# YoungSean/UnseenObjectsWithMeanShift

Measured on AMD Instinct MI355X. Metric: images/sec @640x480 RGB-D, 100 queries, 9 decoder layers; % MFMA roofline, higher is better.
Workload: dtype f32; 1 GPU; configs[1]: batch 8 of 640x480 per GPU, ResNet-50 features -> MSDeformAttn pixel decoder -> 9-layer decoder, 100 q ->~; global_batch=8, per_gpu_batch=8, launch=hipgraph x4: 4 batches of 8 in flight, one graph + stream each, batches_in_flight=4, parallelism=dp1, GPU_MAX_HW_QUEUES=4, visible_gpus=1, rank0_numa=pinned

## Files before the change

include/msm_hip.h:

```cpp
#ifndef MSM_HIP_H
#define MSM_HIP_H

#include <stdint.h>

#ifdef __cplusplus
extern "C" {
#endif

#define MSM_OK 0
#define MSM_E_INVALID (-1)
#define MSM_E_LAUNCH (-2)
#define MSM_E_WORKSPACE (-3)

const char* msm_last_error_string(void);
#define MSM_ABI_VERSION 28
int msm_abi_version(void);

#define MSM_OPT_AUTO (-1)
enum {
    MSM_OPT_MASK_NC = 0,
    MSM_OPT_MASKB_TARGET,
    MSM_OPT_GEMM_TILE,
    MSM_OPT_GEMM_SHALLOW,
    MSM_OPT_ATTN_TARGET,
    MSM_OPT_ATTN_KERNEL,
    MSM_OPT_ATTN_QK_MAX,
    MSM_OPT_ATTN_QKCFG,
    MSM_OPT_CONVIN_NT,
    MSM_OPT_POST_GENERIC,
    MSM_OPT_ENC_NO_COOP,
    MSM_OPT_MSDA_GENERIC,
    MSM_OPT_MS_CHUNK,
    MSM_OPT_MS_NO_PERSISTENT,
    MSM_OPT_ATTN_FUSED_KV,
    MSM_OPT_KV_PIPE,
    MSM_OPT_MASK_KERNEL,
    MSM_OPT_MS_SPLIT_KERNEL,
    MSM_OPT_CONV3_WIDE,
    MSM_OPT_DEC_TILE32,
    MSM_OPT_POST_RESIZE_DIRECT,
    MSM_OPT_COUNT
};
int msm_set_option(int key, int value);
int msm_get_option(int key);

int msm_gemm_f32(const float* A, const float* A2, const float* W, const float* bias, float* C,
                 int M, int N, int K, int batch,
                 int64_t a_sm, int64_t a_sk, int64_t a_sb, int64_t a2_sb, int64_t w_sb,
                 int64_t c_sm, int64_t c_sn, int64_t c_sb, int64_t c_ss,
                 int a_mode, int conv_h, int conv_w, int conv_c,
                 int bias_mode, int act, int split_k, void* stream);

int msm_layernorm_f32(const float* x, const float* parts, int n_parts, int64_t part_stride,
                      const float* bias, const float* g1, const float* b1, int l2norm,
                      const float* g2, const float* b2, float* y, float* y2,
                      int rows, int E, float eps, void* stream);

int msm_groupnorm_stats_f32(const float* x, double* stats, int stats_cleared, int B, int HW, int C, void* stream);
int msm_groupnorm_apply_f32(const float* x, const double* stats, const float* gamma, const float* beta,
                            const float* up, int uh, int uw, int64_t up_batch_stride, float* y,
                            int B, int H, int W, int C, int groups, float eps, int relu, void* stream);

int msm_groupnorm_apply_split(const float* x, const double* stats, const float* gamma, const float* beta,
                              const float* up, int uh, int uw, int64_t up_batch_stride, uint16_t* planes,
                              int B, int H, int W, int C, int groups, float eps, int relu, void* stream);

int msm_groupnorm_apply_f16(const float* x, const double* stats, const float* gamma, const float* beta,
                            const float* up, int uh, int uw, int64_t up_batch_stride, void* y_f16,
                            int B, int H, int W, int C, int groups, float eps, int relu, void* stream);

int msm_groupnorm_apply_nchw_f32(const float* x, const double* stats, const float* gamma, const float* beta, float* y,
                                 int B, int HW, int C, int groups, float eps, int relu, void* stream);

int msm_pos_embed_sine(float* out, int H, int W, int npf, int64_t s_c, int64_t s_p,
                       const float* add_c, float temperature, float scale, void* stream);

int msm_transpose_f32(const float* in, float* out, int B, int R, int C, void* stream);

int msm_l2_normalize_nchw_f32(const float* x, float* y, int B, int C, int HW, float eps, void* stream);

int msm_msda_locations(const float* offsets, const float* logits, const float* reference_points, const int64_t* spatial_shapes,
                       float* sampling_loc, float* attn_weight, int64_t rows, int M, int L, int P, void* stream);

#define MSM_MASK_SPARSE 1
#define MSM_MASK_ROW_ANY_CLEARED 2
#define MSM_MASK_F16 4
int msm_mask_logits_fwd(const float* mask_embed, const float* mask_feat, float* mask_out,
                        uint8_t* attn_out, int32_t* row_any,
                        int B, int Q, int C, int H, int W, int th, int tw, int flags,
                        int64_t embed_ld, const float* qbias, int64_t qbias_ld, void* stream);

int msm_pack_mask_features_bf16(const float* mask_feat, uint16_t* packed, int B, int C, int HW, void* stream);
int msm_pack_mask_features_f16(const float* mask_feat, uint16_t* packed, int B, int C, int HW, void* stream);
int msm_mask_logits_bf16_fwd(const float* mask_embed, const uint16_t* mask_feat_packed, float* mask_out,
                             uint8_t* attn_out, int32_t* row_any,
                             int B, int Q, int C, int H, int W, int th, int tw, int flags,
                             int64_t embed_ld, const float* qbias, int64_t qbias_ld, void* stream);

int msm_pack_mask_features_split(const float* mask_feat, uint16_t* packed, int B, int C, int HW, void* stream);
int msm_mask_logits_split_fwd(const float* mask_embed, const uint16_t* mask_feat_split, float* mask_out,
                              uint8_t* attn_out, int32_t* row_any, int B, int Q, int C, int H, int W, int th, int tw,
                              int flags, int64_t embed_ld, const float* qbias, int64_t qbias_ld, void* stream);

int64_t msm_hypersphere_attn_workspace(int B, int Lq, int S, int heads);
int msm_hypersphere_attn_fwd(const float* q, const float* k, const float* v,
                             const uint8_t* masked, const int32_t* row_any, float* out,
                             int B, int Lq, int S, int heads,
                             int64_t ldq, int64_t q_sb, int64_t ldk, int64_t k_sb,
                             int64_t ldv, int64_t v_sb, float kappa,
                             float* workspace, int64_t workspace_elems, void* stream);
int msm_hypersphere_attn_lp_fwd(const float* q, const void* k, const void* v, int kv_format,
                                const uint8_t* masked, const int32_t* row_any, float* out,
                                int B, int Lq, int S, int heads,
                                int64_t ldq, int64_t q_sb, int64_t ldk, int64_t k_sb,
                                int64_t ldv, int64_t v_sb, float kappa,
                                float* workspace, int64_t workspace_elems, void* stream);

int msm_nchw_to_tokens_f16(const float* in, void* out, int B, int C, int HW, void* stream);
int msm_attn_pack_kv_weights(const float* w, void* packed, int heads, void* stream);
int msm_mask_conv3x3_folded(const void* x_f16, const float* F, int64_t ldf, int64_t f_sb, void* mask_bits, int32_t* row_any, int row_any_cleared,
                            float* logits, int B, int Q, int H, int W, void* stream);
int64_t msm_attn_mask_bits_bytes(int B, int Lq, int S);
int msm_attn_pack_mask_bits(const uint8_t* masked, void* bits, int B, int Lq, int S, void* stream);
int msm_hypersphere_attn_fused_kv_fwd(const float* q, const void* x_f16, const void* w_packed, const float* rowcol, const float* col_v_t,
                                      int score_format, const void* mask_bits, const int32_t* row_any, float* out,
                                      int B, int Lq, int H, int W, int heads, int64_t ldq, int64_t q_sb, float kappa,
                                      float* workspace, int64_t workspace_elems, void* stream);

int msm_msdeform_attn_fwd(const float* value, const int64_t* spatial_shapes,
                          const int64_t* level_start_index, const float* sampling_loc,
                          const float* attn_weight, float* out,
                          int B, int S, int M, int D, int L, int Lq, int P, void* stream);

int msm_msdeform_attn_bwd(const float* value, const int64_t* spatial_shapes,
                          const int64_t* level_start_index, const float* sampling_loc,
                          const float* attn_weight, const float* grad_output,
                          float* grad_value, float* grad_sampling_loc, float* grad_attn_weight,
                          int B, int S, int M, int D, int L, int Lq, int P, void* stream);
int msm_msdeform_attn_fwd_f64(const double* value, const int64_t* spatial_shapes,
                              const int64_t* level_start_index, const double* sampling_loc,
                              const double* attn_weight, double* out,
                              int B, int S, int M, int D, int L, int Lq, int P, void* stream);
int msm_msdeform_attn_bwd_f64(const double* value, const int64_t* spatial_shapes,
                              const int64_t* level_start_index, const double* sampling_loc,
                              const double* attn_weight, const double* grad_output,
                              double* grad_value, double* grad_sampling_loc, double* grad_attn_weight,
                              int B, int S, int M, int D, int L, int Lq, int P, void* stream);

int msm_msdeform_attn_enc_fwd(const float* value, const int64_t* spatial_shapes,
                              const int64_t* level_start_index, const float* proj, float* out,
                              int B, int S, int M, int D, int L, int P, void* stream);

int msm_value_to_head_major_f32(const float* value, float* value_hm, int B, int S, int M, int D, void* stream);
int msm_msdeform_attn_enc_hm_fwd(const float* value_hm, const int64_t* spatial_shapes,
                                 const int64_t* level_start_index, const float* proj, float* out,
// ... 293 lines not shown
```

unseenobjectswithmeanshift_amd/_lib.py:

```python
import ctypes
import os
import re

_HERE = os.path.dirname(os.path.abspath(__file__))
LIB_PATH = os.path.join(_HERE, "libmsm_hip.so")
HEADER_PATH = os.path.join(os.path.dirname(_HERE), "include", "msm_hip.h")

_lib = None
ABI_VERSION = 28

c_f = ctypes.c_void_p
c_p = ctypes.c_void_p
c_i = ctypes.c_int
c_l = ctypes.c_int64
c_fl = ctypes.c_float

_SIGNATURES = {
    "msm_abi_version": (c_i, []),
    "msm_last_error_string": (ctypes.c_char_p, []),
    "msm_set_option": (c_i, [c_i, c_i]),
    "msm_get_option": (c_i, [c_i]),
    "msm_gemm_f32": (c_i, [c_f, c_f, c_f, c_f, c_f, c_i, c_i, c_i, c_i,
                           c_l, c_l, c_l, c_l, c_l, c_l, c_l, c_l, c_l,
                           c_i, c_i, c_i, c_i, c_i, c_i, c_i, c_p]),
    "msm_layernorm_f32": (c_i, [c_f, c_f, c_i, c_l, c_f, c_f, c_f, c_i, c_f, c_f, c_f, c_f, c_i, c_i, c_fl, c_p]),
    "msm_groupnorm_stats_f32": (c_i, [c_f, c_p, c_i, c_i, c_i, c_i, c_p]),
    "msm_groupnorm_apply_f32": (c_i, [c_f, c_p, c_f, c_f, c_f, c_i, c_i, c_l, c_f, c_i, c_i, c_i, c_i, c_i, c_fl, c_i, c_p]),
    "msm_groupnorm_apply_split": (c_i, [c_f, c_p, c_f, c_f, c_f, c_i, c_i, c_l, c_f, c_i, c_i, c_i, c_i, c_i, c_fl, c_i, c_p]),
    "msm_groupnorm_apply_f16": (c_i, [c_f, c_p, c_f, c_f, c_f, c_i, c_i, c_l, c_p, c_i, c_i, c_i, c_i, c_i, c_fl, c_i, c_p]),
    "msm_groupnorm_apply_nchw_f32": (c_i, [c_f, c_p, c_f, c_f, c_f, c_i, c_i, c_i, c_i, c_fl, c_i, c_p]),
    "msm_pos_embed_sine": (c_i, [c_f, c_i, c_i, c_i, c_l, c_l, c_f, c_fl, c_fl, c_p]),
    "msm_transpose_f32": (c_i, [c_f, c_f, c_i, c_i, c_i, c_p]),
    "msm_l2_normalize_nchw_f32": (c_i, [c_f, c_f, c_i, c_i, c_i, c_fl, c_p]),
    "msm_msda_locations": (c_i, [c_f, c_f, c_f, c_p, c_f, c_f, c_l, c_i, c_i, c_i, c_p]),
    "msm_mask_logits_fwd": (c_i, [c_f, c_f, c_f, c_p, c_p, c_i, c_i, c_i, c_i, c_i, c_i, c_i, c_i, c_l, c_f, c_l, c_p]),
    "msm_pool_mask_taps": (c_i, [c_f, c_i, c_i, c_i, c_i, c_p, c_p, c_p, c_p, c_l, c_p]),
    "msm_attn_mask_pooled": (c_i, [c_f, c_l, c_f, c_l, c_f, c_p, c_p, c_i, c_i, c_i, c_i, c_i, c_p]),
    "msm_pack_mask_features_bf16": (c_i, [c_f, c_p, c_i, c_i, c_i, c_p]),
    "msm_pack_mask_features_f16": (c_i, [c_f, c_p, c_i, c_i, c_i, c_p]),
    "msm_mask_logits_bf16_fwd": (c_i, [c_f, c_p, c_f, c_p, c_p, c_i, c_i, c_i, c_i, c_i, c_i, c_i, c_i, c_l, c_f, c_l, c_p]),
    "msm_pack_mask_features_split": (c_i, [c_f, c_p, c_i, c_i, c_i, c_p]),
    "msm_mask_logits_split_fwd": (c_i, [c_f, c_p, c_f, c_p, c_p, c_i, c_i, c_i, c_i, c_i, c_i, c_i, c_i, c_l, c_f, c_l, c_p]),
    "msm_hypersphere_attn_workspace": (c_l, [c_i, c_i, c_i, c_i]),
    "msm_hypersphere_attn_fwd": (c_i, [c_f, c_f, c_f, c_p, c_p, c_f, c_i, c_i, c_i, c_i,
                                       c_l, c_l, c_l, c_l, c_l, c_l, c_fl, c_f, c_l, c_p]),
    "msm_hypersphere_attn_lp_fwd": (c_i, [c_f, c_p, c_p, c_i, c_p, c_p, c_f, c_i, c_i, c_i, c_i,
                                          c_l, c_l, c_l, c_l, c_l, c_l, c_fl, c_f, c_l, c_p]),
    "msm_hypersphere_attn_bwd_workspace": (c_l, [c_i, c_i, c_i]),
    "msm_hypersphere_attn_bwd": (c_i, [c_f, c_f, c_f, c_p, c_p, c_f, c_f, c_f, c_f, c_i, c_i, c_i, c_i,
                                       c_l, c_l, c_l, c_l, c_l, c_l, c_fl, c_f, c_l, c_p]),
    "msm_msdeform_attn_fwd": (c_i, [c_f, c_p, c_p, c_f, c_f, c_f, c_i, c_i, c_i, c_i, c_i, c_i, c_i, c_p]),
    "msm_msdeform_attn_bwd": (c_i, [c_f, c_p, c_p, c_f, c_f, c_f, c_f, c_f, c_f, c_i, c_i, c_i, c_i, c_i, c_i, c_i, c_p]),
    "msm_msdeform_attn_fwd_f64": (c_i, [c_f, c_p, c_p, c_f, c_f, c_f, c_i, c_i, c_i, c_i, c_i, c_i, c_i, c_p]),
    "msm_msdeform_attn_bwd_f64": (c_i, [c_f, c_p, c_p, c_f, c_f, c_f, c_f, c_f, c_f, c_i, c_i, c_i, c_i, c_i, c_i, c_i, c_p]),
    "msm_msdeform_attn_enc_fwd": (c_i, [c_f, c_p, c_p, c_f, c_f, c_i, c_i, c_i, c_i, c_i, c_i, c_p]),
    "msm_encoder_block_stream_floats": (c_l, [c_i, c_i]),
    "msm_value_to_head_major_f32": (c_i, [c_f, c_f, c_i, c_i, c_i, c_i, c_p]),
    "msm_msdeform_attn_enc_hm_fwd": (c_i, [c_f, c_p, c_p, c_f, c_f, c_i, c_i, c_i, c_i, c_i, c_i, c_p]),
    "msm_msda_pack_proj": (c_i, [c_f, c_f, c_f, c_f, c_i, c_i, c_i, c_p]),
    "msm_msdeform_attn_enc_fused_fwd": (c_i, [c_f, c_p, c_p, c_f, c_f, c_f, c_f, c_f, c_i, c_i, c_i, c_i, c_i, c_i, c_p]),
    "msm_encoder_block_fwd": (c_i, [c_f, c_f, c_f, c_f, c_f, c_f, c_f, c_f, c_i, c_i, c_i, c_i, c_i, c_fl, c_p]),
    "msm_encoder_block_split_stream_bytes": (c_l, [c_i, c_i]),
    "msm_encoder_block_split_fwd": (c_i, [c_f, c_f, c_p, c_f, c_f, c_f, c_f, c_f, c_i, c_i, c_i, c_i, c_i, c_fl, c_p]),
    "msm_encoder_block_lp_stream_bytes": (c_l, [c_i, c_i]),
    "msm_encoder_block_lp_fwd": (c_i, [c_f, c_f, c_p, c_f, c_f, c_f, c_f, c_f, c_i, c_i, c_i, c_i, c_i, c_fl, c_p]),
    "msm_encoder_block_hm_stream_bytes": (c_l, [c_i, c_i]),
    "msm_encoder_block_hm_small_floats": (c_i, [c_i]),
    "msm_encoder_block_hm_fwd": (c_i, [c_p, c_f, c_p, c_f, c_f, c_f, c_p, c_p, c_i, c_i, c_i, c_fl, c_i, c_p]),
    "msm_msdeform_attn_enc_lp_fwd": (c_i, [c_p, c_p, c_p, c_p, c_p, c_i, c_i, c_i, c_i, c_i, c_i, c_p]),
    "msm_msdeform_attn_enc_lp_fused_fwd": (c_i, [c_p, c_p, c_p, c_f, c_f, c_p, c_f, c_p, c_i, c_i, c_i, c_i, c_i, c_i, c_p]),
    "msm_f32_to_f16": (c_i, [c_f, c_p, c_l, c_p]),
    "msm_bias_act_nhwc": (c_i, [c_p, c_p, c_p, c_i, c_l, c_i, c_i, c_p]),
    "msm_nhwc_to_nchw_f32": (c_i, [c_p, c_f, c_i, c_i, c_i, c_i, c_p]),
    "msm_ucn_embedding_tail": (c_i, [c_f, c_f, c_f, c_i, c_i, c_i, c_i, c_i, c_i, c_fl, c_p]),
    "msm_f32_to_f16_rows": (c_i, [c_f, c_p, c_i, c_l, c_l, c_p]),
    "msm_kv_project_f32": (c_i, [c_f, c_f, c_f, c_f, c_i, c_i, c_i, c_i, c_i, c_l, c_i, c_p]),
    "msm_kv_project_multi_f32": (c_i, [c_i, c_p, c_p, c_p, c_p, c_p, c_p, c_p, c_p, c_i, c_i, c_i, c_p]),
    "msm_kv_project_multi_bf16": (c_i, [c_i, c_p, c_p, c_p, c_p, c_p, c_p, c_p, c_p, c_i, c_i, c_i, c_i, c_p]),
    "msm_kv_project_multi_split": (c_i, [c_i, c_p, c_p, c_p, c_p, c_p, c_p, c_p, c_p, c_i, c_i, c_i, c_p]),
    "msm_tokens_proj_nchw_f32": (c_i, [c_f, c_f, c_f, c_p, c_f, c_f, c_i, c_fl, c_i, c_f, c_i, c_i, c_i, c_i, c_p]),
    "msm_dec_pack_weight": (c_i, [c_f, c_f, c_i, c_i, c_p]),
    "msm_dec_post_cross": (c_i, [c_f] * 12 + [c_i, c_i, c_i, c_fl, c_p]),
    "msm_dec_post_self": (c_i, [c_f] * 9 + [c_i, c_f, c_f, c_i, c_i, c_i, c_fl, c_p]),
    "msm_dec_heads": (c_i, [c_f, c_f, c_i, c_f, c_f, c_f, c_i] + [c_f] * 15 + [c_p, c_i, c_i, c_i, c_fl, c_p]),
    "msm_dec_pack_weight_bf16": (c_i, [c_f, c_p, c_i, c_i, c_p]),
    "msm_dec_post_cross_bf16": (c_i, [c_f, c_f, c_f, c_p, c_f, c_f, c_f, c_p, c_f, c_f, c_f, c_f] + [c_i, c_i, c_i, c_fl, c_p]),
    "msm_dec_post_self_bf16": (c_i, [c_f, c_f, c_p, c_f, c_f, c_f, c_p, c_f, c_p] + [c_i, c_f, c_f, c_i, c_i, c_i, c_fl, c_p]),
    "msm_dec_heads_bf16": (c_i, [c_f, c_f, c_i, c_f, c_f, c_f, c_i, c_f, c_f, c_p, c_f, c_p, c_f, c_p, c_f, c_p, c_f, c_f] + [c_f] * 4 +
                           [c_p, c_i, c_i, c_i, c_fl, c_p]),
    "msm_nchw_to_tokens_f16": (c_i, [c_f, c_p, c_i, c_i, c_i, c_p]),
    "msm_mask_conv3x3_folded": (c_i, [c_p, c_f, c_l, c_l, c_p, c_p, c_i, c_f, c_i, c_i, c_i, c_i, c_p]),
    "msm_attn_pack_kv_weights": (c_i, [c_f, c_p, c_i, c_p]),
    "msm_attn_mask_bits_bytes": (c_l, [c_i, c_i, c_i]),
    "msm_attn_pack_mask_bits": (c_i, [c_p, c_p, c_i, c_i, c_i, c_p]),
    "msm_hypersphere_attn_fused_kv_fwd": (c_i, [c_f, c_p, c_p, c_f, c_f, c_i, c_p, c_p, c_f, c_i, c_i, c_i, c_i, c_i, c_l, c_l, c_fl, c_f, c_l, c_p]),
    "msm_dec_pack_weight_f16": (c_i, [c_f, c_p, c_i, c_i, c_p]),
    "msm_dec_post_cross_f16": (c_i, [c_f, c_f, c_f, c_p, c_f, c_f, c_f, c_p, c_f, c_f, c_f, c_f] + [c_i, c_i, c_i, c_fl, c_p]),
    "msm_dec_post_self_f16": (c_i, [c_f, c_f, c_p, c_f, c_f, c_f, c_p, c_f, c_p] + [c_i, c_f, c_f, c_i, c_i, c_i, c_fl, c_p]),
    "msm_dec_heads_f16": (c_i, [c_f, c_f, c_i, c_f, c_f, c_f, c_i, c_f, c_f, c_p, c_f, c_p, c_f, c_p, c_f, c_p, c_f, c_f] + [c_f] * 4 +
                          [c_p, c_i, c_i, c_i, c_fl, c_p]),
    "msm_dec_heads_mask": (c_i, [c_f, c_f, c_i, c_f, c_f, c_f, c_i, c_f, c_f, c_p, c_f, c_p, c_f, c_p, c_f, c_p, c_f, c_f] + [c_f] * 4 +
                           [c_f, c_i, c_i, c_p, c_p, c_i, c_i, c_i, c_i, c_fl, c_p]),
    "msm_dec_pack_weight_bf16x2": (c_i, [c_f, c_p, c_i, c_i, c_p]),
    "msm_dec_post_cross_bf16x2": (c_i, [c_f, c_f, c_f, c_p, c_f, c_f, c_f, c_p, c_f, c_f, c_f, c_f] + [c_i, c_i, c_i, c_fl, c_p]),
    "msm_dec_post_self_bf16x2": (c_i, [c_f, c_f, c_p, c_f, c_f, c_f, c_p, c_f, c_p] + [c_i, c_f, c_f, c_i, c_i, c_i, c_fl, c_p]),
    "msm_dec_heads_bf16x2": (c_i, [c_f, c_f, c_i, c_f, c_f, c_f, c_i, c_f, c_f, c_p, c_f, c_p, c_f, c_p, c_f, c_p, c_f, c_f] + [c_f] * 4 +
                             [c_p, c_i, c_i, c_i, c_fl, c_p]),
    "msm_l2_prefetch": (c_i, [c_p, c_p, c_i, c_p]),
    "msm_dec_set_prefetch": (c_i, [c_p, c_p, c_i]),
    "msm_ms_seed_workspace": (c_l, [c_i]),
    "msm_ms_select_seeds": (c_i, [c_f, c_i, c_i, c_i, c_l, c_f, c_p, c_f, c_l, c_i, c_p]),
    "msm_ms_hill_climb_workspace": (c_l, [c_i, c_i]),
    "msm_ms_hill_climb": (c_i, [c_f, c_i, c_i, c_f, c_i, c_fl, c_i, c_f, c_l, c_p]),
# ... 1 lines not shown
    "msm_ms_hill_climb_split": (c_i, [c_f, c_i, c_i, c_f, c_i, c_fl, c_i, c_f, c_l, c_p]),
    "msm_ms_bf16_rows": (c_l, [c_i]),
    "msm_ms_pack_bf16": (c_i, [c_f, c_i, c_i, c_p, c_p]),
    "msm_ms_select_seeds_bf16": (c_i, [c_p, c_f, c_i, c_i, c_i, c_l, c_f, c_p, c_f, c_l, c_i, c_p]),
    "msm_ms_hill_climb_bf16": (c_i, [c_p, c_i, c_i, c_f, c_i, c_fl, c_i, c_f, c_l, c_p]),
    "msm_ms_assign": (c_i, [c_f, c_i, c_i, c_f, c_i, c_p, c_p, c_p, c_i, c_p]),
    "msm_ms_connected_components": (c_i, [c_f, c_i, c_i, c_fl, c_p, c_p, c_p]),
    "msm_ms_relabel_largest_zero": (c_i, [c_p, c_i, c_p, c_i, c_p, c_p]),
    "msm_ms_seed_batched_workspace": (c_l, [c_i, c_i]),
    "msm_ms_select_seeds_batched": (c_i, [c_f, c_i, c_i, c_i, c_i, c_p, c_f, c_p, c_f, c_l, c_i, ctypes.c_uint64, c_p]),
    "msm_ms_hill_climb_batched_workspace": (c_l, [c_i, c_i, c_i]),
    "msm_ms_hill_climb_batched": (c_i, [c_f, c_i, c_i, c_i, c_f, c_i, c_fl, c_i, c_f, c_l, c_p]),
    "msm_ms_assign_batched": (c_i, [c_f, c_i, c_i, c_i, c_f, c_i, c_p, c_p, c_p, c_i, c_p]),
    "msm_ms_connected_components_batched": (c_i, [c_f, c_i, c_i, c_i, c_fl, c_p, c_p, c_p]),
    "msm_ms_relabel_largest_zero_batched": (c_i, [c_p, c_i, c_i, c_p, c_i, c_p, c_p]),
    "msm_topk_class_scores": (c_i, [c_f, c_i, c_i, c_i, c_i, c_f, c_p, c_p, c_p]),
    "msm_topk_class_scores_gather": (c_i, [c_f, c_i, c_i, c_i, c_i, c_f, c_p, c_p, c_f, c_l, c_i, c_f, c_p]),
    "msm_conv1x1_in_f32": (c_i, [c_f, c_f, c_f, c_f, c_l, c_p, c_i, c_i, c_i, c_i, c_p]),
    "msm_conv1x1_in_multi_f32": (c_i, [c_i, c_p, c_p, c_p, c_p, c_p, c_f, c_l, c_p, c_i, c_i, c_p]),
    "msm_conv1x1_in_multi_lp": (c_i, [c_i, c_p, c_p, c_p, c_p, c_p, c_f, c_l, c_p, c_i, c_i, c_p]),
    "msm_conv1x1_in_multi_wide": (c_i, [c_i, c_p, c_p, c_p, c_p, c_p, c_f, c_l, c_p, c_i, c_i, c_p]),
    "msm_conv1x1_in_lp": (c_i, [c_f, c_p, c_f, c_f, c_l, c_p, c_i, c_i, c_i, c_i, c_p]),
    "msm_conv3x3_c64_f32": (c_i, [c_f, c_f, c_f, c_p, c_i, c_i, c_i, c_i, c_p]),
    "msm_conv3x3_c64_bf16": (c_i, [c_f, c_f, c_f, c_p, c_i, c_i, c_i, c_i, c_p]),
    "msm_conv3x3_c64_f16": (c_i, [c_f, c_f, c_f, c_p, c_i, c_i, c_i, c_i, c_p]),
    "msm_conv3x3_c64_f16h": (c_i, [c_p, c_f, c_f, c_p, c_i, c_i, c_i, c_i, c_p]),
    "msm_conv3x3_c64_nchw_f16": (c_i, [c_f, c_f, c_f, c_f, c_i, c_i, c_i, c_i, c_p]),
    "msm_conv3x3_c64_split": (c_i, [c_f, c_f, c_f, c_p, c_i, c_i, c_i, c_i, c_p]),
    "msm_conv3x3_c64_nchw_f32": (c_i, [c_f, c_f, c_f, c_f, c_i, c_i, c_i, c_i, c_p]),
    "msm_conv3x3_c64_nchw_bf16": (c_i, [c_f, c_f, c_f, c_f, c_i, c_i, c_i, c_i, c_p]),
    "msm_encoder_prologue_stream_floats": (c_l, [c_i]),
    "msm_encoder_prologue_fwd": (c_i, [c_f, c_p, c_f, c_p, c_i, c_i, c_fl, c_f, c_f, c_f, c_f, c_p, c_p, c_i, c_i, c_i, c_i, c_i, c_p]),
    "msm_encoder_prologue_hm_weight_bytes": (c_l, []),
    "msm_encoder_prologue_hm_fwd": (c_i, [c_f, c_p, c_f, c_p, c_i, c_i, c_fl, c_p, c_f, c_f, c_f, c_p, c_p, c_i, c_i, c_p]),
    "msm_label_stats": (c_i, [c_f, c_f, c_p, c_f, c_p, c_i, c_i, c_i, c_i, c_p]),
    "msm_label_image": (c_i, [c_f, c_f, c_f, c_i, c_i, c_i, c_i, c_p]),
    "msm_crop_resize": (c_i, [c_f, c_f, c_f, c_p, c_f, c_f, c_f, c_i, c_i, c_i, c_i, c_p]),
    "msm_paste_labels": (c_i, [c_f, c_p, c_p, c_p, c_f, c_i, c_i, c_i, c_i, c_p]),
    "msm_mask_nms_workspace": (c_l, [c_i, c_i, c_i, c_i]),
    "msm_mask_nms": (c_i, [c_f, c_f, c_p, c_fl, c_f, c_f, c_f, c_p, c_p, c_p, c_l, c_i, c_i, c_i, c_i, c_p]),
    "msm_ingest_frames": (c_i, [c_p, c_p, c_i, c_fl, c_f, c_f, c_f, c_f, c_i, c_i, c_i, c_i, c_i, c_i, c_p]),
    "msm_instance_postprocess_workspace": (c_l, [c_i, c_i, c_i, c_i]),
    "msm_eval_counts_workspace": (c_l, [c_i]),
    "msm_eval_counts": (c_i, [c_f, c_f, c_p, c_p, c_l, c_i, c_i, c_i, c_i, c_i, c_p]),
    "msm_match_cost": (c_i, [c_p, c_p, c_p, c_f, c_f, c_i, c_i, c_i, c_i, c_i, c_i, c_i, c_i, c_i, c_i, c_i,
                             c_fl, c_fl, c_fl, c_p]),
    "msm_point_loss_workspace": (c_l, [c_i, c_i]),
    "msm_point_loss_fwd": (c_i, [c_p, c_p, c_p, c_f, c_f, c_f, c_p, c_p, c_l, c_i, c_i, c_i, c_i, c_i, c_i, c_i, c_i,
                                 c_i, c_i, c_i, c_fl, c_p]),
    "msm_point_loss_bwd": (c_i, [c_p, c_p, c_p, c_f, c_f, c_p, c_l, c_f, c_i, c_i, c_i, c_i, c_i, c_i, c_i, c_i,
                                 c_i, c_i, c_i, c_fl, c_i, c_p]),
    "msm_instance_postprocess": (c_i, [c_f, c_p, c_f, c_f, c_f, c_f, c_i, c_i, c_i, c_i, c_i, c_i, c_i, c_i, c_i, c_f, c_p]),
    "msm_instance_postprocess_resized": (c_i, [c_f, c_p, c_f, c_f, c_f, c_f] + [c_i] * 11 + [c_f, c_p]),
}


def declared_symbols():
    with open(HEADER_PATH) as f:
        src = f.read()
    src = re.sub(r"/\*.*?\*/", "", src, flags=re.S)
    return sorted(set(re.findall(r"\b(msm_[a-z0-9_]+)\s*\(", src)))


def lib():
    global _lib
    if _lib is None:
        if not os.path.exists(LIB_PATH):
            raise RuntimeError(
                f"{LIB_PATH} is missing: build it with `python -c 'import __graft_entry__ as g; g.build()'` "
                "(hipcc --offload-arch=gfx950). There is no CPU fallback for the HIP hot path.")
        L = ctypes.CDLL(LIB_PATH)
        for name, (res, args) in _SIGNATURES.items():
            fn = getattr(L, name)
            fn.restype = res
            fn.argtypes = args
        if L.msm_abi_version() != ABI_VERSION:
            raise RuntimeError(f"{LIB_PATH} has ABI {L.msm_abi_version()}, these bindings need {ABI_VERSION}: rebuild it")
        _lib = L
    return _lib


OPTIONS = ("MASK_NC", "MASKB_TARGET", "GEMM_TILE", "GEMM_SHALLOW", "ATTN_TARGET", "ATTN_KERNEL", "ATTN_QK_MAX", "ATTN_QKCFG",
           "CONVIN_NT", "POST_GENERIC", "ENC_NO_COOP", "MSDA_GENERIC", "MS_CHUNK", "MS_NO_PERSISTENT", "ATTN_FUSED_KV", "KV_PIPE", "MASK_KERNEL",
           "MS_SPLIT_KERNEL", "CONV3_WIDE", "DEC_TILE32", "POST_RESIZE_DIRECT")
OPT_AUTO = -1


def set_option(name, value=OPT_AUTO):
    key = OPTIONS.index(name)
    old = lib().msm_get_option(key)
    check(lib().msm_set_option(key, int(value)), "msm_set_option")
    if old != int(value):
        from ._plan import bump_plan_epoch
        bump_plan_epoch()
    return old


class option:

    def __init__(self, name, value):
        self.name, self.value = name, value

    def __enter__(self):
        self.old = set_option(self.name, self.value)
        return self

    def __exit__(self, *exc):
        set_option(self.name, self.old)
        return False


class CallTimer:

    def __init__(self):
        self.records = []
        self._saved = {}

    def __enter__(self):
        import torch
        L = lib()
        for name, (_, args) in _SIGNATURES.items():
            if not args or args[-1] is not c_p or name.endswith("_workspace"):
                continue
            fn = getattr(L, name)
            self._saved[name] = fn

            def wrapped(*a, _fn=fn, _name=name):
                e0, e1 = torch.cuda.Event(enable_timing=True), torch.cuda.Event(enable_timing=True)
                e0.record()
                rc = _fn(*a)
                e1.record()
                self.records.append((_name, e0, e1))
                return rc

            setattr(L, name, wrapped)
        return self

    def __exit__(self, *exc):
        L = lib()
        for name, fn in self._saved.items():
            setattr(L, name, fn)
        self._saved = {}
        return False

    def durations(self):
        out = {}
        for name, e0, e1 in self.records:
            out.setdefault(name, []).append(e0.elapsed_time(e1))
        return out


def check(rc, what):
    if rc != 0:
        msg = lib().msm_last_error_string()
        raise RuntimeError(f"{what} failed (code {rc}): {msg.decode() if msg else ''}")
```

unseenobjectswithmeanshift_amd/csrc/mask_logits.hip:

```cpp
#include <stdlib.h>

#include <type_traits>

#include "bf16.h"
#include "common.h"

namespace msm {

constexpr int QB = 7;
constexpr int QCH = QB * 16;
#ifndef MSM_MASK_KU
#define MSM_MASK_KU 4
#endif
#ifndef MSM_WRITE_AUX
#define MSM_WRITE_AUX 0
#endif
#ifndef MSM_MASK_MW
#define MSM_MASK_MW 8
#endif
constexpr int KU = MSM_MASK_KU;
constexpr int MW = MSM_MASK_MW;

typedef unsigned int u32x2 __attribute__((ext_vector_type(2)));

#ifdef MSM_MASK_TS
__device__ unsigned long long g_mask_ts[256 * 8 * 16];
#define MASK_TS(slot)                                                                                          \
    if (lane == 0 && blockIdx.y == 0 && (int)(blockIdx.z * gridDim.x + blockIdx.x) < 256 && (slot) < 16)       \
        g_mask_ts[((blockIdx.z * gridDim.x + blockIdx.x) * 8 + wave) * 16 + (slot)] = wall_clock64();
#define MASK_TSC(slot)                                                                                         \
    if (lane == 0 && blockIdx.y == 0 && (int)(blockIdx.z * gridDim.x + blockIdx.x) < 256 && (slot) < 16)       \
        g_mask_ts[((blockIdx.z * gridDim.x + blockIdx.x) * 8 + wave) * 16 + (slot)] = clock64();
#else
#define MASK_TS(slot)
#define MASK_TSC(slot)
#endif

template <int NC>
struct Cols {
    float v[NC];
};
template <int NC>
__device__ __forceinline__ Cols<NC> ld_cols(__amdgpu_buffer_rsrc_t rsrc, unsigned voff, unsigned soff) {
    Cols<NC> c;
    if constexpr (NC == 2) {
        const u32x2 t = __builtin_amdgcn_raw_buffer_load_b64(rsrc, voff, soff, 0);
        c.v[0] = __uint_as_float(t.x);
        c.v[1] = __uint_as_float(t.y);
    } else {
        c.v[0] = __uint_as_float(__builtin_amdgcn_raw_buffer_load_b32(rsrc, voff, soff, 0));
    }
    return c;
}

template <int POOL, int NC>
struct PixMap {
    static constexpr bool PERM = (POOL == 8 && NC == 1);
    __device__ static __forceinline__ int load_col(int i) {
        if constexpr (PERM) {
            const int g = i >> 2, r = i & 3;
            return (g >> 1) * 8 + (int)((((g & 1) ? 0x7610u : 0x5243u) >> (4 * r)) & 15u);
        } else {
            return NC * i;
        }
    }
    __device__ static __forceinline__ int out_col(int lq, int j) {
        if constexpr (PERM) return load_col(lq * 4 + j);
        else return 4 * NC * lq + j;
    }
};

template <int NC>
__device__ __forceinline__ float acc_val(const f32x4 (&acc)[QB][2 * NC], int m, int row, int j) {
    if constexpr (NC == 2) return acc[m][row * 2 + (j & 1)][j >> 1];
    else return acc[m][row][j];
}

template <int POOL, bool WRITE, int NC, bool DO_WRITE = true, bool DO_ATTN = true, bool R4 = false>
__device__ __forceinline__ void mask_tile_epilogue(const f32x4 (&acc)[QB][2 * NC], float* __restrict__ mask_out,
                                                   uint8_t* __restrict__ attn_out, int* __restrict__ any_flags, int b, int Q,
                                                   int q0, int H, int W, int th, int tw, int ytop, int ybot, int c0, int lj, int lq) {
    using PM = PixMap<POOL, NC>;
    constexpr int NP = 4 * NC;
    int ql = lj;
    asm volatile("" : "+v"(ql));
    const int xb = c0 + NP * lq;
    if constexpr (WRITE && DO_WRITE) {
#pragma unroll
        for (int m = 0; m < QB; ++m) {
            const bool rem = R4 && m == QB - 1;
            const int pg = rem ? (ql >> 2) : lq;
            const int xb = c0 + NP * pg;
            const bool vec = !PM::PERM && xb + NP <= W && (W & 3) == 0;
            const int q = rem ? q0 + m * 16 + (ql & 3) : q0 + m * 16 + ql;
            if (q >= Q || (rem && lq != 0)) continue;
            float* o = mask_out + ((int64_t)b * Q + q) * ((int64_t)H * W);
#pragma unroll
            for (int row = 0; row < 2; ++row) {
                const int y = row ? ybot : ytop;
                if (y < 0 || y >= H) continue;
                float* orow = o + (int64_t)y * W;
                if (vec) {
#pragma unroll
                    for (int j = 0; j < NP; j += 4)
                        *reinterpret_cast<float4*>(orow + xb + j) = make_float4(acc_val<NC>(acc, m, row, j), acc_val<NC>(acc, m, row, j + 1),
                                                                               acc_val<NC>(acc, m, row, j + 2), acc_val<NC>(acc, m, row, j + 3));
                } else {
#pragma unroll
                    for (int j = 0; j < NP; ++j) {
                        const int x = c0 + PM::out_col(pg, j);
                        if (x < W) orow[x] = acc_val<NC>(acc, m, row, j);
                    }
                }
            }
        }
    }
    if constexpr (!DO_ATTN) {
        return;
    } else if constexpr (POOL == 1) {
        const int HW = H * W;
        const bool vec = xb + NP <= W && (W & 3) == 0;
#pragma unroll
        for (int m = 0; m < QB; ++m) {
            const int q = q0 + m * 16 + ql;
            if (q >= Q) continue;
            uint8_t* o = attn_out + ((int64_t)b * Q + q) * HW;
            bool any = false;
#pragma unroll
            for (int row = 0; row < 2; ++row) {
                const int y = row ? ybot : ytop;
                if (y < 0 || y >= H) continue;
#pragma unroll
                for (int j0 = 0; j0 < NP; j0 += 4) {
                    uint32_t w = 0;
#pragma unroll
                    for (int j = 0; j < 4; ++j) w |= (acc_val<NC>(acc, m, row, j0 + j) < 0.f ? 1u : 0u) << (8 * j);
                    if (vec) {
                        *reinterpret_cast<uint32_t*>(o + (int64_t)y * W + xb + j0) = w;
                        any |= w != 0x01010101u;
                    } else {
#pragma unroll
                        for (int j = 0; j < 4; ++j) {
                            const int x = xb + j0 + j;
                            if (x < W) { o[(int64_t)y * W + x] = (uint8_t)((w >> (8 * j)) & 1u); any |= ((w >> (8 * j)) & 1u) == 0u; }
                        }
                    }
                }
            }
            if (any) any_flags[q - q0] = 1;
        }
    } else if constexpr (POOL != 0) {
        if (!((ytop >= 0) && (ybot < H) && ((ytop % POOL) == POOL / 2 - 1))) return;
        const int ty = ytop / POOL;
        if (ty >= th) return;
        constexpr int NT = PM::PERM ? 1 : (NP / POOL > 0 ? NP / POOL : 1);
        constexpr int J0 = PM::PERM ? 0 : POOL / 2 - 1;
        constexpr int JS = PM::PERM ? 0 : POOL;
        const bool lane_tap = PM::PERM ? ((lq & 1) == 0) : true;
        const int tx0 = PM::PERM ? (c0 / 8 + (lq >> 1)) : (xb / POOL);
        static_assert(PM::PERM || NP >= POOL, "a lane must hold whole taps");
        const bool vec = NT == 4 ? ((tw & 3) == 0 && tx0 + 4 <= tw) : (NT == 2 ? ((tw & 1) == 0 && tx0 + 2 <= tw) : (tx0 < tw));
#pragma unroll
        for (int m = 0; m < QB; ++m) {
            uint32_t w = 0;
#pragma unroll
            for (int t = 0; t < NT; ++t) {
                const int jl = J0 + t * JS;
                const float s = (acc_val<NC>(acc, m, 0, jl) + acc_val<NC>(acc, m, 0, jl + 1)) +
                                (acc_val<NC>(acc, m, 1, jl) + acc_val<NC>(acc, m, 1, jl + 1));
                w |= (s < 0.f ? 1u : 0u) << (8 * t);
            }
            const int q = q0 + m * 16 + ql;
            if (q < Q && lane_tap) {
                uint8_t* o = attn_out + ((int64_t)b * Q + q) * (th * tw) + ty * tw + tx0;
                if (vec) {
                    if constexpr (NT == 4) *reinterpret_cast<uint32_t*>(o) = w;
                    else if constexpr (NT == 2) *reinterpret_cast<uint16_t*>(o) = (uint16_t)w;
                    else *o = (uint8_t)w;
                    constexpr uint32_t ALL = NT == 4 ? 0x01010101u : (NT == 2 ? 0x0101u : 0x01u);
                    if (w != ALL) any_flags[q - q0] = 1;
                } else {
#pragma unroll
                    for (int t = 0; t < NT; ++t)
                        if (tx0 + t < tw) {
                            o[t] = (uint8_t)((w >> (8 * t)) & 1u);
                            if (((w >> (8 * t)) & 1u) == 0u) any_flags[q - q0] = 1;
                        }
                }
            }
            __builtin_amdgcn_sched_barrier(0);
        }
    }
}

template <int POOL, bool WRITE, int NC>
struct MaskEpiConst {
    unsigned aoff[QB];
    unsigned moff[QB];
    unsigned anyv[QB];
    __amdgpu_buffer_rsrc_t arsrc, mrsrc;
    bool attn_fast, write_fast;
};

__device__ __forceinline__ float add1(float a, float b) {
    float r;
    asm("v_add_f32 %0, %1, %2" : "=v"(r) : "v"(a), "v"(b));
    return r;
}
__device__ __forceinline__ unsigned neg_bit(float x) { return __float_as_uint(x) >> 31; }

__device__ __forceinline__ void* uniform_ptr64(const void* p) {
    const uint64_t u = (uint64_t)p;
    return (void*)(((uint64_t)(unsigned)__builtin_amdgcn_readfirstlane((int)(u >> 32)) << 32) |
                   (uint64_t)(unsigned)__builtin_amdgcn_readfirstlane((int)(unsigned)u));
}

template <int POOL, bool WRITE, int NC>
__device__ __forceinline__ void mask_epi_init(MaskEpiConst<POOL, WRITE, NC>& k, float* mask_out, uint8_t* attn_out, int b, int Q, int q0,
                                              int H, int W, int th, int tw, int lj, int lq, bool r4 = false) {
    using PM = PixMap<POOL, NC>;
    constexpr int NP = 4 * NC;
    const int HW = H * W;
    const int TT = POOL == 1 ? HW : th * tw;
    constexpr int NT = PM::PERM ? 1 : (POOL == 1 ? NP : (NP / (POOL > 0 ? POOL : 1) > 0 ? NP / (POOL > 0 ? POOL : 1) : 1));
#pragma unroll
    for (int m = 0; m < QB; ++m) {
        const bool rem = r4 && m == QB - 1;
        const int pgl = rem ? (lj >> 2) : lq;
        const int q = rem ? q0 + m * 16 + (lj & 3) : q0 + m * 16 + lj;
        const int lane_key = POOL == 1 ? NP * pgl : (PM::PERM ? (pgl >> 1) : (NP * pgl) / (POOL > 0 ? POOL : 1));
        const bool lane_on = (PM::PERM ? ((pgl & 1) == 0) : true) && (!rem || lq == 0);
        k.aoff[m] = (lane_on && q < Q) ? (unsigned)(q * TT + lane_key) : 0xF0000000u;
        k.moff[m] = (q < Q && (!rem || lq == 0)) ? (unsigned)((q * HW + NP * pgl) * 4) : 0xF0000000u;
        k.anyv[m] = 0u;
    }
    if constexpr (POOL != 0)
        k.arsrc = __builtin_amdgcn_make_buffer_rsrc(uniform_ptr64(attn_out + (int64_t)b * Q * TT), 0, Q * TT, 0x00020000);
    if constexpr (WRITE)
        k.mrsrc = __builtin_amdgcn_make_buffer_rsrc(uniform_ptr64(mask_out + (int64_t)b * Q * HW), 0, Q * HW * 4, 0x00020000);
    const int keys_row = POOL == 1 ? W : tw;
    k.attn_fast = POOL != 0 && (NT == 4 || NT == 8 ? (keys_row & 3) == 0 : (NT == 2 ? (keys_row & 1) == 0 : true)) && (int64_t)Q * TT < 0xF0000000ll;
    k.write_fast = WRITE && !PM::PERM && (W & 3) == 0 && (int64_t)Q * HW * 4 < 0xF0000000ll;
}

typedef unsigned int u32x4 __attribute__((ext_vector_type(4)));

template <int POOL, bool WRITE, int NC, bool DO_WRITE, bool DO_ATTN, bool R4_PARTIAL = false>
__device__ __forceinline__ void mask_tile_epilogue_fast(const f32x4 (&acc)[QB][2 * NC], MaskEpiConst<POOL, WRITE, NC>& k, int H, int W, int tw,
                                                        int ytop, int ybot, int c0) {
    using PM = PixMap<POOL, NC>;
    constexpr int NP = 4 * NC;
    if constexpr (WRITE && DO_WRITE) {
        static_assert(NC == 1, "mask writes take 2 x 16 tiles");
#pragma unroll
        for (int row = 0; row < 2; ++row) {
            const int y = row ? ybot : ytop;
            if (y < 0 || y >= H) continue;
            const unsigned soff = (unsigned)(y * W + c0) * 4u;
#pragma unroll
            for (int m = 0; m < QB; ++m)
#pragma unroll
                for (int j = 0; j < NP; j += 4)
                    __builtin_amdgcn_raw_buffer_store_b128(u32x4{__float_as_uint(acc_val<NC>(acc, m, row, j)), __float_as_uint(acc_val<NC>(acc, m, row, j + 1)),
                                                                 __float_as_uint(acc_val<NC>(acc, m, row, j + 2)), __float_as_uint(acc_val<NC>(acc, m, row, j + 3))},
                                                           k.mrsrc, k.moff[m] + 4u * j, soff, MSM_WRITE_AUX);
        }
    }
    if constexpr (!DO_ATTN || POOL == 0) {
        return;
    } else if constexpr (POOL == 1) {
#pragma unroll
        for (int row = 0; row < 2; ++row) {
            const int y = row ? ybot : ytop;
            if (y < 0 || y >= H) continue;
            const unsigned soff = (unsigned)(y * W + c0);
#pragma unroll
            for (int m = 0; m < QB; ++m)
#pragma unroll
                for (int j0 = 0; j0 < NP; j0 += 4) {
                    unsigned w = 0;
#pragma unroll
                    for (int j = 0; j < 4; ++j) w |= acc_val<NC>(acc, m, row, j0 + j) < 0.f ? (1u << (8 * j)) : 0u;
                    __builtin_amdgcn_raw_buffer_store_b32(w, k.arsrc, k.aoff[m] + j0, soff, 0);
                    k.anyv[m] |= w ^ 0x01010101u;
                }
        }
    } else {
        if (!((ytop >= 0) && (ybot < H) && ((ytop % POOL) == POOL / 2 - 1))) return;
        constexpr int NT = PM::PERM ? 1 : NP / POOL;
        constexpr int J0 = PM::PERM ? 0 : POOL / 2 - 1;
        constexpr int JS = PM::PERM ? 0 : POOL;
        static_assert(PM::PERM || NP >= POOL, "a lane must hold whole taps");
        const unsigned soff = (unsigned)((ytop / POOL) * tw + c0 / POOL);
#pragma unroll
        for (int m = 0; m < QB; ++m) {
            unsigned w = 0;
#pragma unroll
            for (int t = 0; t < NT; ++t) {
                const int jl = J0 + t * JS;
                float s = add1(add1(acc_val<NC>(acc, m, 0, jl), acc_val<NC>(acc, m, 0, jl + 1)),
                               add1(acc_val<NC>(acc, m, 1, jl), acc_val<NC>(acc, m, 1, jl + 1)));
                if constexpr (R4_PARTIAL) {
                    if (m == QB - 1) {
                        s = sum_lane_rows(s);
                    }
                }
                w = t == 0 ? neg_bit(s) : (w | (neg_bit(s) << (8 * t)));
            }
#ifndef MSM_EPI_AUX
#define MSM_EPI_AUX 0
#endif
            if constexpr (NT == 4) {
#ifndef MSM_EPI_NOSTORE
                __builtin_amdgcn_raw_buffer_store_b32(w, k.arsrc, k.aoff[m], soff, MSM_EPI_AUX);
#endif
                k.anyv[m] |= w ^ 0x01010101u;
            } else if constexpr (NT == 2) {
#ifndef MSM_EPI_NOSTORE
                __builtin_amdgcn_raw_buffer_store_b16((unsigned short)w, k.arsrc, k.aoff[m], soff, MSM_EPI_AUX);
#endif
                k.anyv[m] |= w ^ 0x0101u;
            } else {
#ifndef MSM_EPI_NOSTORE
                __builtin_amdgcn_raw_buffer_store_b8((unsigned char)w, k.arsrc, k.aoff[m], soff, MSM_EPI_AUX);
#endif
                k.anyv[m] |= w ^ 0x01u;
            }
        }
    }
}

template <int POOL, bool WRITE, int NC>
__device__ __forceinline__ void mask_epi_flush(const MaskEpiConst<POOL, WRITE, NC>& k, int* __restrict__ any_flags, int lj, bool r4 = false) {
    if constexpr (POOL != 0) {
#pragma unroll
        for (int m = 0; m < QB; ++m)
            if (k.anyv[m] != 0u && k.aoff[m] != 0xF0000000u) any_flags[m * 16 + ((r4 && m == QB - 1) ? (lj & 3) : lj)] = 1;
    }
}

template <int POOL, bool WRITE, int NC, int D, bool R4 = false>
__global__ __launch_bounds__(MW * 64) void mask_logits_kernel(const float* __restrict__ emb, const float* __restrict__ feat,
                                                          float* __restrict__ mask_out, uint8_t* __restrict__ attn_out,
                                                          int32_t* __restrict__ row_any, int Q, int C, int H, int W,
                                                          int th, int tw, int ypar, int n_rowpairs, int rp_step,
                                                          int rp_first, int feat_bytes, int64_t emb_ld,
                                                          const float* __restrict__ qbias, int64_t qbias_ld) {
    extern __shared__ __attribute__((aligned(16))) float Es[];
    constexpr int TW = 16 * NC;
    constexpr int NA = 2 * NC;
    const int SE = C + 2;
    const int b = blockIdx.z, qc = blockIdx.y;
    const int q0 = qc * QCH;
    const int tid = threadIdx.x, lane = tid & 63;
    const int wave = __builtin_amdgcn_readfirstlane(tid >> 6);
    const int lj = lane & 15, lq = lane >> 4;
    const int HW = H * W;
    MASK_TS(0)

    const int ctiles = (W + TW - 1) / TW;
    const int ntiles = n_rowpairs * ctiles;
    const __amdgpu_buffer_rsrc_t rsrc = __builtin_amdgcn_make_buffer_rsrc(uniform_ptr64(feat + (int64_t)b * C * HW), 0, feat_bytes, 0x00020000);

    const int slots = gridDim.x * MW;
    const int full_rounds = ntiles / slots;
    const int left = ntiles - full_rounds * slots;
    const int left_slot = (wave >> 2) * ((int)gridDim.x * 4) + (int)blockIdx.x * 4 + (wave & 3);
    const int my_tiles = full_rounds + (left_slot < left ? 1 : 0);
    auto tile_of = [&](int it) {
        return (it < full_rounds) ? it * slots + (int)blockIdx.x * MW + wave : full_rounds * slots + left_slot;
    };
    auto tile_voffs = [&](int t, unsigned& vtop, unsigned& vbot) {
        const int rp = t / ctiles, ct = t - rp * ctiles;
        const int ytop = ypar + 2 * (rp_first + rp * rp_step);
        const int ybot = ytop + 1;
        const int c = ct * TW + PixMap<POOL, NC>::load_col(lj);
        const int cl = c < W ? c : 0;
        vtop = (unsigned)(((int64_t)lq * HW + (int64_t)max(ytop, 0) * W + cl) * 4);
        vbot = (unsigned)(((int64_t)lq * HW + (int64_t)min(ybot, H - 1) * W + cl) * 4);
    };
    Cols<NC> tR[D][KU], bR[D][KU];
    auto load_group = [&](Cols<NC>(&t)[KU], Cols<NC>(&bt)[KU], int kbase, unsigned vtop, unsigned vbot) {
#pragma unroll
        for (int u = 0; u < KU; ++u) {
            const unsigned soff = (unsigned)(kbase + u * 4) * (unsigned)HW * 4u;
            t[u] = ld_cols<NC>(rsrc, vtop, soff);
            bt[u] = ld_cols<NC>(rsrc, vbot, soff);
        }
    };
    const float* eb = emb + ((int64_t)b * Q + q0) * emb_ld;
    const int c4n = C >> 2;
    const bool colwise = (MW * 64) % c4n == 0 && 4 * ((MW * 64) / c4n) >= QCH;
    const int rpp = colwise ? (MW * 64) / c4n : 1, r0 = colwise ? tid / c4n : 0, c4 = colwise ? (tid - r0 * c4n) * 4 : 0;
    float4 ev[4];
    if (colwise) {
#pragma unroll
        for (int i = 0; i < 4; ++i) {
            const int r = r0 + i * rpp;
            ev[i] = make_float4(0.f, 0.f, 0.f, 0.f);
            if (r < QCH && q0 + r < Q) ev[i] = *reinterpret_cast<const float4*>(eb + (int64_t)r * emb_ld + c4);
        }
    }
    unsigned voff_top = 0, voff_bot = 0;
    tile_voffs(tile_of(0), voff_top, voff_bot);
    if (my_tiles > 0) {
#pragma unroll
        for (int d = 0; d < D; ++d) load_group(tR[d], bR[d], d * (4 * KU), voff_top, voff_bot);
    }
    if (colwise) {
#pragma unroll
        for (int i = 0; i < 4; ++i) {
            const int r = r0 + i * rpp;
            if (r < QCH) {
                float2* d = reinterpret_cast<float2*>(&Es[r * SE + c4]);
                d[0] = make_float2(ev[i].x, ev[i].y);
                d[1] = make_float2(ev[i].z, ev[i].w);
            }
        }
    } else {
        for (int idx = tid; idx < QCH * c4n; idx += MW * 64) {
            const int r = idx / c4n, cc4 = (idx - r * c4n) * 4;
            float4 v = make_float4(0.f, 0.f, 0.f, 0.f);
            if (q0 + r < Q) v = *reinterpret_cast<const float4*>(eb + (int64_t)r * emb_ld + cc4);
            float2* d = reinterpret_cast<float2*>(&Es[r * SE + cc4]);
            d[0] = make_float2(v.x, v.y);
            d[1] = make_float2(v.z, v.w);
        }
    }
    float* qb = Es + QCH * SE;
    int* any_flags = reinterpret_cast<int*>(qb + QCH);
    for (int r = tid; r < QCH; r += MW * 64) {
        qb[r] = (qbias && q0 + r < Q) ? qbias[((int64_t)b * Q + q0 + r) * qbias_ld] : 0.f;
        any_flags[r] = 0;
    }
    __syncthreads();
    MASK_TS(1)

    constexpr int NB4 = NC == 1 ? QB : 1;
    f32x4 bias4[NB4];
    if constexpr (NC == 1) {
#pragma unroll
        for (int m = 0; m < QB; ++m) {
            float q_b = qb[m * 16 + lj];
            if (R4 && m == QB - 1) q_b = lq == 0 ? qb[m * 16 + (lj & 3)] : 0.f;
            bias4[m] = f32x4{q_b, q_b, q_b, q_b};
        }
    }
    static_assert(!R4 || NC == 1, "the 4-query block exists for 2 x 16 tiles only");
    MaskEpiConst<POOL, WRITE, NC> epi;
    mask_epi_init<POOL, WRITE, NC>(epi, mask_out, attn_out, b, Q, q0, H, W, th, tw, lj, lq, R4);

    const int G = C / (4 * KU);
#ifndef MSM_MASK_NOPRIO
    if (wave < 4) __builtin_amdgcn_s_setprio(3);
#endif
    for (int it = 0; it < my_tiles; ++it) {
        const int t = tile_of(it);
        const int rp = t / ctiles, ct = t - rp * ctiles;
        const int ytop = ypar + 2 * (rp_first + rp * rp_step);
        const int ybot = ytop + 1;
        const int c0 = ct * TW;
        unsigned nvoff_top, nvoff_bot;
        tile_voffs(tile_of(min(it + 1, my_tiles - 1)), nvoff_top, nvoff_bot);

        f32x4 acc[QB][NA];
        auto compute_group = [&](auto first, const Cols<NC>(&t_)[KU], const Cols<NC>(&bt)[KU], int kbase) {
#pragma unroll
            for (int u = 0; u < KU; ++u) {
                const float* er = &Es[lj * SE + kbase + u * 4 + lq];
#pragma unroll
                for (int m = 0; m < QB; ++m) {
                    if constexpr (R4) {
                        if (m == QB - 1) {
                            const float a4 = Es[(m * 16 + (lj & 3)) * SE + kbase + u * 4 + lq];
                            if (decltype(first)::value && u == 0) {
                                acc[m][0] = __builtin_amdgcn_mfma_f32_4x4x1f32(t_[u].v[0], a4, bias4[m], 0, 0, 0);
                                acc[m][1] = __builtin_amdgcn_mfma_f32_4x4x1f32(bt[u].v[0], a4, bias4[m], 0, 0, 0);
                            } else {
                                acc[m][0] = __builtin_amdgcn_mfma_f32_4x4x1f32(t_[u].v[0], a4, acc[m][0], 0, 0, 0);
                                acc[m][1] = __builtin_amdgcn_mfma_f32_4x4x1f32(bt[u].v[0], a4, acc[m][1], 0, 0, 0);
                            }
                            continue;
                        }
                    }
                    const float a = er[m * 16 * SE];
#pragma unroll
                    for (int cc = 0; cc < NC; ++cc) {
                        if (decltype(first)::value && u == 0) {
                            f32x4 c4;
                            if constexpr (NC == 1) {
                                c4 = bias4[m];
                            } else {
                                const float q_b = qb[m * 16 + lj];
                                c4 = f32x4{q_b, q_b, q_b, q_b};
                            }
                            acc[m][cc] = mfma16(t_[u].v[cc], a, c4);
                            acc[m][NC + cc] = mfma16(bt[u].v[cc], a, c4);
                        } else {
                            acc[m][cc] = mfma16(t_[u].v[cc], a, acc[m][cc]);
                            acc[m][NC + cc] = mfma16(bt[u].v[cc], a, acc[m][NC + cc]);
                        }
                    }
                }
            }
        };
        auto ring_pass = [&](auto first, int gb) {
#pragma unroll
            for (int d = 0; d < D; ++d) {
                const int g = gb + d;
                if (d == 0) compute_group(first, tR[d], bR[d], g * (4 * KU));
                else compute_group(std::false_type{}, tR[d], bR[d], g * (4 * KU));
                __builtin_amdgcn_sched_barrier(0);
                const bool more = g + D < G;
                load_group(tR[d], bR[d], (more ? g + D : g + D - G) * (4 * KU), more ? voff_top : nvoff_top, more ? voff_bot : nvoff_bot);
                __builtin_amdgcn_sched_barrier(0);
            }
        };
        ring_pass(std::true_type{}, 0);
        for (int gb = D; gb < G; gb += D) ring_pass(std::false_type{}, gb);
        voff_top = nvoff_top;
        voff_bot = nvoff_bot;
        MASK_TS(2 + 3 * it)
#ifdef MSM_MASK_TS
        {
            float dep = acc[QB - 1][NA - 1][3];
            asm volatile("v_mov_b32 %0, %0" : "+v"(dep));
            MASK_TS(3 + 3 * it)
        }
#endif
        const bool inside = c0 + TW <= W;
        if constexpr (R4) {
            mask_tile_epilogue_fast<POOL, WRITE, NC, false, true, true>(acc, epi, H, W, tw, ytop, ybot, c0);
            if constexpr (WRITE) {
#pragma unroll
                for (int row = 0; row < 2; ++row)
#pragma unroll
                    for (int r = 0; r < 4; ++r) {
                        float v = acc[QB - 1][row][r];
                        v = sum_lane_rows(v);
                        acc[QB - 1][row][r] = v;
                    }
            }
        }
        if constexpr (WRITE) {
            static_assert(NC == 1, "mask writes take 2 x 16 tiles (see mask_tile_epilogue_fast)");
            if (inside && epi.write_fast) mask_tile_epilogue_fast<POOL, WRITE, NC, true, false>(acc, epi, H, W, tw, ytop, ybot, c0);
            else mask_tile_epilogue<POOL, WRITE, NC, true, false, R4>(acc, mask_out, attn_out, any_flags, b, Q, q0, H, W, th, tw, ytop, ybot, c0, lj, lq);
        }
        if constexpr (!R4) {
            if (inside && epi.attn_fast) mask_tile_epilogue_fast<POOL, WRITE, NC, false, true>(acc, epi, H, W, tw, ytop, ybot, c0);
            else mask_tile_epilogue<POOL, WRITE, NC, false, true>(acc, mask_out, attn_out, any_flags, b, Q, q0, H, W, th, tw, ytop, ybot, c0, lj, lq);
        }
        MASK_TS(4 + 3 * it)
    }
    if constexpr (POOL != 0) {
        mask_epi_flush<POOL, WRITE, NC>(epi, any_flags, lj, R4);
        __syncthreads();
        for (int r = tid; r < QCH; r += MW * 64)
            if (any_flags[r] && q0 + r < Q) row_any[(int64_t)b * Q + q0 + r] = 1;
    }
}

constexpr int BKS = 16;

__device__ __forceinline__ unsigned short f2bf(float x) {
    const unsigned int u = __float_as_uint(x);
    return (unsigned short)((u + 0x7fffu + ((u >> 16) & 1u)) >> 16);
}

__device__ __forceinline__ unsigned short f2h(float x) {
    return __builtin_bit_cast(unsigned short, (_Float16)__builtin_amdgcn_fmed3f(x, -65504.f, 65504.f));
}
typedef _Float16 f16x4m __attribute__((ext_vector_type(4)));
template <int POOL, bool WRITE, int NKS, bool F16 = false>
__global__ __launch_bounds__(MW * 64) void mask_logits_bf16_kernel(const float* __restrict__ emb, const unsigned short* __restrict__ featp,
                                                               float* __restrict__ mask_out, uint8_t* __restrict__ attn_out,
                                                               int32_t* __restrict__ row_any, int Q, int C, int H, int W, int th,
                                                               int tw, int ypar, int n_rowpairs, int rp_step, int rp_first,
                                                               int feat_bytes, int64_t emb_ld, const float* __restrict__ qbias,
                                                               int64_t qbias_ld) {
    extern __shared__ __attribute__((aligned(16))) unsigned short Eb[];
    const int SEb = C + 8;
    const int b = blockIdx.z, qc = blockIdx.y;
    const int q0 = qc * QCH;
    const int tid = threadIdx.x, lane = tid & 63;
    const int wave = __builtin_amdgcn_readfirstlane(tid >> 6);
    const int lj = lane & 15, lq = lane >> 4;
    const int HW = H * W;
    const int nks = C / 16;

    const float* eb = emb + ((int64_t)b * Q + q0) * emb_ld;
    float* qb = reinterpret_cast<float*>(Eb + QCH * SEb);
    int* any_flags = reinterpret_cast<int*>(qb + QCH);
    for (int r = tid; r < QCH; r += MW * 64) {
        qb[r] = (qbias && q0 + r < Q) ? qbias[((int64_t)b * Q + q0 + r) * qbias_ld] : 0.f;
        any_flags[r] = 0;
    }
    for (int idx = tid; idx < QCH * (C / 4); idx += MW * 64) {
        const int r = idx / (C / 4), c4 = (idx - r * (C / 4)) * 4;
        float4 v = make_float4(0.f, 0.f, 0.f, 0.f);
        if (q0 + r < Q) v = *reinterpret_cast<const float4*>(eb + (int64_t)r * emb_ld + c4);
        u32x2 pk;
        if constexpr (F16) {
            pk.x = (unsigned)f2h(v.x) | ((unsigned)f2h(v.y) << 16);
            pk.y = (unsigned)f2h(v.z) | ((unsigned)f2h(v.w) << 16);
        } else {
            pk.x = (unsigned)f2bf(v.x) | ((unsigned)f2bf(v.y) << 16);
            pk.y = (unsigned)f2bf(v.z) | ((unsigned)f2bf(v.w) << 16);
        }
        *reinterpret_cast<u32x2*>(&Eb[r * SEb + c4]) = pk;
    }
    __syncthreads();

    const int ctiles = (W + 15) / 16;
    const int ntiles = n_rowpairs * ctiles;
    const uint64_t fbu = (uint64_t)(featp + (int64_t)b * C * HW);
    const uint64_t fbs = ((uint64_t)(unsigned)__builtin_amdgcn_readfirstlane((int)(fbu >> 32)) << 32) |
                         (uint64_t)(unsigned)__builtin_amdgcn_readfirstlane((int)(unsigned)fbu);
    const __amdgpu_buffer_rsrc_t rsrc = __builtin_amdgcn_make_buffer_rsrc((void*)fbs, 0, feat_bytes, 0x00020000);

    const int slots = gridDim.x * MW;
    const int full_rounds = ntiles / slots;
    const int left = ntiles - full_rounds * slots;
// ... 221 lines not shown
        __syncthreads();
        for (int r = tid; r < QCH; r += MW * 64)
            if (any_flags[r] && q0 + r < Q) row_any[(int64_t)b * Q + q0 + r] = 1;
    }
}

__global__ __launch_bounds__(256) void pack_mask_features_split_kernel(const float* __restrict__ in, unsigned short* __restrict__ out,
                                                                       int64_t total, int C8, int HW) {
    for (int64_t i = (int64_t)blockIdx.x * 256 + threadIdx.x; i < total; i += (int64_t)gridDim.x * 256) {
        const int p = (int)(i % HW);
        const int64_t r = i / HW;
        const int64_t bimg = r / C8;
        const int kg = (int)(r - bimg * C8);
        const float* src = in + (r * 8) * HW + p;
        float v[8];
#pragma unroll
        for (int j = 0; j < 8; ++j) v[j] = src[(int64_t)j * HW];
        const Split3 a = split3(v[0], v[1], v[2], v[3]), c = split3(v[4], v[5], v[6], v[7]);
        const Split3x8 s8 = join(a, c);
        unsigned short* dst = out + ((bimg * 3 * C8 + kg) * (int64_t)HW + p) * 8;
        *reinterpret_cast<u32x4b*>(dst) = __builtin_bit_cast(u32x4b, s8.h);
        *reinterpret_cast<u32x4b*>(dst + (int64_t)C8 * HW * 8) = __builtin_bit_cast(u32x4b, s8.m);
        *reinterpret_cast<u32x4b*>(dst + 2 * (int64_t)C8 * HW * 8) = __builtin_bit_cast(u32x4b, s8.l);
    }
}

}

using namespace msm;

static int mask_embed_check(const char* who, const float* mask_embed, int64_t& embed_ld, const float* qbias, int64_t& qbias_ld, int C) {
    if (embed_ld == 0) embed_ld = C;
    if (qbias && qbias_ld == 0) qbias_ld = 1;
    MSM_REQUIRE(embed_ld >= C && embed_ld % 4 == 0 && (((uintptr_t)mask_embed) & 15) == 0, "%s: mask_embed row stride %lld must be >= C, a multiple of 4, base 16-byte aligned",
                who, (long long)embed_ld);
    MSM_REQUIRE(!qbias || qbias_ld >= 1, "%s: bad qbias stride", who);
    return MSM_OK;
}

extern "C" int msm_mask_logits_fwd(const float* mask_embed, const float* mask_feat, float* mask_out,
                                   uint8_t* attn_out, int32_t* row_any, int B, int Q, int C, int H, int W,
                                   int th, int tw, int flags, int64_t embed_ld, const float* qbias, int64_t qbias_ld, void* stream) {
    const int sparse = flags & MSM_MASK_SPARSE;
    MSM_REQUIRE(mask_embed && mask_feat, "msm_mask_logits_fwd: null input");
    MSM_REQUIRE(mask_out || attn_out, "msm_mask_logits_fwd: nothing to produce");
    MSM_REQUIRE(B > 0 && Q > 0 && H > 1 && W > 1, "msm_mask_logits_fwd: bad sizes");
    MSM_REQUIRE(C % 32 == 0 && C >= 32 && C <= 320, "msm_mask_logits_fwd: C=%d must be a multiple of 32 and <= 320", C);
    if (int rc = mask_embed_check("msm_mask_logits_fwd", mask_embed, embed_ld, qbias, qbias_ld, C)) return rc;
    MSM_REQUIRE(W % 2 == 0 && H % 2 == 0, "msm_mask_logits_fwd: H=%d W=%d must be even", H, W);
    MSM_REQUIRE((int64_t)C * H * W * 4 < (int64_t)1 << 31, "msm_mask_logits_fwd: one image of mask_feat must be < 2 GiB");
    MSM_REQUIRE((((uintptr_t)mask_embed) & 15) == 0 && (((uintptr_t)mask_feat) & 7) == 0 &&
                    (!mask_out || (((uintptr_t)mask_out) & 7) == 0),
                "msm_mask_logits_fwd: misaligned pointer");
    int pool = 0;
    if (attn_out) {
        MSM_REQUIRE(row_any, "msm_mask_logits_fwd: row_any required with attn_out");
        MSM_REQUIRE(th > 0 && tw > 0 && H % th == 0 && W % tw == 0 && H / th == W / tw,
                    "msm_mask_logits_fwd: target %dx%d incompatible with %dx%d", th, tw, H, W);
        pool = H / th;
        MSM_REQUIRE(pool == 1 || pool == 2 || pool == 4 || pool == 8, "msm_mask_logits_fwd: pool factor %d not in {1,2,4,8}", pool);
    }
    hipStream_t st = (hipStream_t)stream;
    if (attn_out && !(flags & MSM_MASK_ROW_ANY_CLEARED)) MSM_CHECK_HIP(hipMemsetAsync(row_any, 0, sizeof(int32_t) * (size_t)B * Q, st));

    int ypar = 0, n_rowpairs = H / 2, rp_step = 1, rp_first = 0;
    if (pool == 4 || pool == 8) {
        ypar = -1;
        n_rowpairs = H / 2 + 1;
        if (sparse && !mask_out) {
            rp_step = pool / 2;
            rp_first = pool / 4;
            n_rowpairs = H / pool;
        }
    }
    const int qchunks = cdiv(Q, QCH);
    const int64_t t32 = (int64_t)n_rowpairs * cdiv(W, 32) * B * qchunks;
    const int64_t t16 = (int64_t)n_rowpairs * cdiv(W, 16) * B * qchunks;
    const double cost32 = (double)cdiv(t32, 1024), cost16 = 0.5 * (double)cdiv(t16, 1024);
    int nc = (cost16 * 1.04 < cost32 || (cost16 <= cost32 && cost32 < 3.0)) ? 1 : 2;
    if (const int o = opt(MSM_OPT_MASK_NC); o != MSM_OPT_AUTO) nc = o == 1 ? 1 : 2;
    if (mask_out) nc = 1;
    const int ctiles = cdiv(W, 16 * nc);
    const int ntiles = n_rowpairs * ctiles;
    int wg_per = cdiv(ntiles, MW);
    const size_t lds = sizeof(float) * ((size_t)QCH * (C + 2) + 2 * QCH);
    const int target = cdiv(256, B * qchunks);
    if (wg_per > target) wg_per = max(target, 1);
    dim3 grid(wg_per, qchunks, B), block(MW * 64);
    typedef void (*kern_t)(const float*, const float*, float*, uint8_t*, int32_t*, int, int, int, int, int, int, int, int, int, int, int, int64_t,
                           const float*, int64_t);
    kern_t kern;
    const bool wr = mask_out != nullptr;
    const bool r4 = nc == 1 && Q == 100 && W % 16 == 0 && (int64_t)Q * H * W * 4 < 0xF0000000ll && opt(MSM_OPT_MASK_KERNEL) != 5 &&
                    (pool == 0 || pool == 2 || pool == 4 || pool == 8);
#define MASK_PICK(P)                                                                                                   \
    (wr ? (r4 ? (kern_t)mask_logits_kernel<P, true, 1, 2, true> : (kern_t)mask_logits_kernel<P, true, 1, 2>)             \
        : (nc == 2 ? (kern_t)mask_logits_kernel<P, false, 2, 2>                                                          \
                   : (r4 ? (kern_t)mask_logits_kernel<P, false, 1, 2, true> : (kern_t)mask_logits_kernel<P, false, 1, 2>)))
    switch (pool) {
        case 0: kern = r4 ? (kern_t)mask_logits_kernel<0, true, 1, 2, true> : (kern_t)mask_logits_kernel<0, true, 1, 2>; break;
        case 1: kern = MASK_PICK(1); break;
        case 2: kern = MASK_PICK(2); break;
        case 4: kern = MASK_PICK(4); break;
        default: kern = MASK_PICK(8); break;
    }
#undef MASK_PICK
    MSM_CHECK_HIP((hipError_t)ensure_dynamic_lds((const void*)kern, lds));
    hipLaunchKernelGGL(kern, grid, block, lds, st, mask_embed, mask_feat, mask_out, attn_out, row_any, Q, C, H, W, th, tw,
                       ypar, n_rowpairs, rp_step, rp_first, (int)((int64_t)C * H * W * 4), embed_ld, qbias, qbias_ld);
    MSM_CHECK_LAUNCH("msm_mask_logits_fwd");
    return MSM_OK;
}

#ifdef MSM_MASK_TS
extern "C" int msm_debug_mask_ts(unsigned long long* host_out) {
    return (int)hipMemcpyFromSymbol(host_out, HIP_SYMBOL(msm::g_mask_ts), sizeof(unsigned long long) * 256 * 8 * 16);
}
#endif

static int pack_mask_features_16(const char* who, const float* mask_feat, uint16_t* packed, int B, int C, int HW, bool f16, void* stream) {
    MSM_REQUIRE(mask_feat && packed, "%s: null pointer", who);
    MSM_REQUIRE(B > 0 && HW > 0 && C > 0 && C % 4 == 0, "%s: C=%d must be a multiple of 4", who, C);
    MSM_REQUIRE((((uintptr_t)packed) & 7) == 0, "%s: packed must be 8-byte aligned", who);
    const int64_t total = (int64_t)B * (C / 4) * HW;
    const dim3 grid((unsigned)min((int64_t)4096, (total + 255) / 256));
    if (f16) hipLaunchKernelGGL(pack_mask_features_bf16_kernel<true>, grid, dim3(256), 0, (hipStream_t)stream, mask_feat, packed, total, C / 4, HW);
    else hipLaunchKernelGGL(pack_mask_features_bf16_kernel<false>, grid, dim3(256), 0, (hipStream_t)stream, mask_feat, packed, total, C / 4, HW);
    MSM_CHECK_LAUNCH(who);
    return MSM_OK;
}
extern "C" int msm_pack_mask_features_bf16(const float* mask_feat, uint16_t* packed, int B, int C, int HW, void* stream) {
    return pack_mask_features_16("msm_pack_mask_features_bf16", mask_feat, packed, B, C, HW, false, stream);
}
extern "C" int msm_pack_mask_features_f16(const float* mask_feat, uint16_t* packed, int B, int C, int HW, void* stream) {
    return pack_mask_features_16("msm_pack_mask_features_f16", mask_feat, packed, B, C, HW, true, stream);
}

extern "C" int msm_mask_logits_bf16_fwd(const float* mask_embed, const uint16_t* mask_feat_packed, float* mask_out,
                                        uint8_t* attn_out, int32_t* row_any, int B, int Q, int C, int H, int W, int th, int tw,
                                        int flags, int64_t embed_ld, const float* qbias, int64_t qbias_ld, void* stream) {
    const int sparse = flags & MSM_MASK_SPARSE;
    MSM_REQUIRE(mask_embed && mask_feat_packed, "msm_mask_logits_bf16_fwd: null input");
    MSM_REQUIRE(mask_out || attn_out, "msm_mask_logits_bf16_fwd: nothing to produce");
    MSM_REQUIRE(B > 0 && Q > 0 && H > 1 && W > 1, "msm_mask_logits_bf16_fwd: bad sizes");
    MSM_REQUIRE(C % 16 == 0 && C >= 16 && C <= 16 * BKS, "msm_mask_logits_bf16_fwd: C=%d must be a multiple of 16 and <= %d", C, 16 * BKS);
    if (int rc = mask_embed_check("msm_mask_logits_bf16_fwd", mask_embed, embed_ld, qbias, qbias_ld, C)) return rc;
    MSM_REQUIRE(W % 2 == 0 && H % 2 == 0, "msm_mask_logits_bf16_fwd: H=%d W=%d must be even", H, W);
    MSM_REQUIRE((int64_t)C * H * W * 2 < (int64_t)1 << 31, "msm_mask_logits_bf16_fwd: one image of mask_feat must be < 2 GiB");
    MSM_REQUIRE((((uintptr_t)mask_embed) & 15) == 0 && (((uintptr_t)mask_feat_packed) & 7) == 0, "msm_mask_logits_bf16_fwd: misaligned pointer");
    int pool = 0;
    if (attn_out) {
        MSM_REQUIRE(row_any, "msm_mask_logits_bf16_fwd: row_any required with attn_out");
        MSM_REQUIRE(th > 0 && tw > 0 && H % th == 0 && W % tw == 0 && H / th == W / tw,
                    "msm_mask_logits_bf16_fwd: target %dx%d incompatible with %dx%d", th, tw, H, W);
        pool = H / th;
        MSM_REQUIRE(pool == 1 || pool == 2 || pool == 4 || pool == 8, "msm_mask_logits_bf16_fwd: pool factor %d not in {1,2,4,8}", pool);
    }
    hipStream_t st = (hipStream_t)stream;
    if (attn_out && !(flags & MSM_MASK_ROW_ANY_CLEARED)) MSM_CHECK_HIP(hipMemsetAsync(row_any, 0, sizeof(int32_t) * (size_t)B * Q, st));
    int ypar = 0, n_rowpairs = H / 2, rp_step = 1, rp_first = 0;
    if (pool == 4 || pool == 8) {
        ypar = -1;
        n_rowpairs = H / 2 + 1;
        if (sparse && !mask_out) {
            rp_step = pool / 2;
            rp_first = pool / 4;
            n_rowpairs = H / pool;
        }
    }
    const int qchunks = cdiv(Q, QCH);
    const int ntiles = n_rowpairs * cdiv(W, 16);
    int wg_per = cdiv(ntiles, MW);
    const int tgt_total = opt(MSM_OPT_MASKB_TARGET) > 0 ? opt(MSM_OPT_MASKB_TARGET) : 256;
    const int target = cdiv(tgt_total, B * qchunks);
    if (wg_per > target) wg_per = max(target, 1);
    dim3 grid(wg_per, qchunks, B), block(MW * 64);
    const size_t lds = sizeof(unsigned short) * (size_t)QCH * (C + 8) + sizeof(float) * 2 * QCH;
    typedef void (*kern_t)(const float*, const unsigned short*, float*, uint8_t*, int32_t*, int, int, int, int, int, int, int, int, int, int, int,
                           int64_t, const float*, int64_t);
    const bool wr = mask_out != nullptr;
    kern_t kern;
    const bool f16 = (flags & MSM_MASK_F16) != 0;
#define MASKB_PICK_T(P, WR, NK) (f16 ? (kern_t)mask_logits_bf16_kernel<P, WR, NK, true> : (kern_t)mask_logits_bf16_kernel<P, WR, NK, false>)
#define MASKB_PICK(P) (C <= 64 ? (wr ? MASKB_PICK_T(P, true, 4) : MASKB_PICK_T(P, false, 4)) : (wr ? MASKB_PICK_T(P, true, BKS) : MASKB_PICK_T(P, false, BKS)))
    switch (pool) {
        case 0: kern = C <= 64 ? MASKB_PICK_T(0, true, 4) : MASKB_PICK_T(0, true, BKS); break;
        case 1: kern = MASKB_PICK(1); break;
        case 2: kern = MASKB_PICK(2); break;
        case 4: kern = MASKB_PICK(4); break;
// ... 81 lines not shown
```

unseenobjectswithmeanshift_amd/csrc/norm.hip:

```cpp
#include "bf16.h"
#include "common.h"

namespace msm {

template <int N>
__device__ __forceinline__ float tree_sum(const float* v) {
    if constexpr (N == 1) return v[0];
    else return tree_sum<N / 2>(v) + tree_sum<N / 2>(v + N / 2);
}

template <int VPT>
__global__ __launch_bounds__(256) void layernorm_kernel(const float* __restrict__ x, const float* __restrict__ parts,
                                                        int n_parts, int64_t part_stride,
                                                        const float* __restrict__ bias,
                                                        const float* __restrict__ g1, const float* __restrict__ b1,
                                                        int l2norm, const float* __restrict__ g2,
                                                        const float* __restrict__ b2, float* __restrict__ y,
                                                        float* __restrict__ y2, int rows, float eps) {
    constexpr int E = VPT * 64;
    const int lane = threadIdx.x & 63;
    const int row = blockIdx.x * 4 + (threadIdx.x >> 6);
    if (row >= rows) return;
    const int64_t base = (int64_t)row * E;
    float v[VPT];
// ... 128 lines not shown
        v.y = (v.y - mn[c + 1]) * sc[c + 1] + sh[c + 1];
        v.z = (v.z - mn[c + 2]) * sc[c + 2] + sh[c + 2];
        v.w = (v.w - mn[c + 3]) * sc[c + 3] + sh[c + 3];
        if (up) {
            const int yy = p / W, xx = p - yy * W;
            int y0, y1, x0, x1;
            float ly, lx;
            bilin_src(yy, uh, H, y0, y1, ly);
            bilin_src(xx, uw, W, x0, x1, lx);
            const float* ub = up + (int64_t)b * up_sb + c;
            const float4 v00 = *reinterpret_cast<const float4*>(ub + ((int64_t)y0 * uw + x0) * C);
            const float4 v01 = *reinterpret_cast<const float4*>(ub + ((int64_t)y0 * uw + x1) * C);
            const float4 v10 = *reinterpret_cast<const float4*>(ub + ((int64_t)y1 * uw + x0) * C);
            const float4 v11 = *reinterpret_cast<const float4*>(ub + ((int64_t)y1 * uw + x1) * C);
            const float hy = 1.f - ly, hx = 1.f - lx;
            v.x += hy * (hx * v00.x + lx * v01.x) + ly * (hx * v10.x + lx * v11.x);
            v.y += hy * (hx * v00.y + lx * v01.y) + ly * (hx * v10.y + lx * v11.y);
            v.z += hy * (hx * v00.z + lx * v01.z) + ly * (hx * v10.z + lx * v11.z);
            v.w += hy * (hx * v00.w + lx * v01.w) + ly * (hx * v10.w + lx * v11.w);
        }
        if (relu) {
            v.x = fmaxf(v.x, 0.f); v.y = fmaxf(v.y, 0.f); v.z = fmaxf(v.z, 0.f); v.w = fmaxf(v.w, 0.f);
        }
        if (planes && h16) {
            *reinterpret_cast<u32x2b*>(planes + ((int64_t)b * HW + p) * C + c) = pack4h(v.x, v.y, v.z, v.w);
        } else if (planes) {
            const Split3 t3 = split3(v.x, v.y, v.z, v.w);
            uint16_t* pb = planes + ((int64_t)b * HW + p) * C + c;
            *reinterpret_cast<u32x2b*>(pb) = __builtin_bit_cast(u32x2b, t3.h);
            *reinterpret_cast<u32x2b*>(pb + plane_stride) = __builtin_bit_cast(u32x2b, t3.m);
            *reinterpret_cast<u32x2b*>(pb + 2 * plane_stride) = __builtin_bit_cast(u32x2b, t3.l);
        } else {
            *reinterpret_cast<float4*>(yb + (int64_t)p * C + c) = v;
        }
    }
}

__global__ __launch_bounds__(256) void gn_apply_nchw_kernel(const float* __restrict__ x, const double* __restrict__ stats,
                                                            const float* __restrict__ gamma, const float* __restrict__ beta,
                                                            float* __restrict__ y, int HW, int C, int groups, float eps, int relu) {
    extern __shared__ float gl[];
    float *sc = gl, *sh = gl + C, *mn = gl + 2 * C, *tile = gl + 3 * C;
    const int b = blockIdx.y, p0 = blockIdx.x * 64;
    const int cpg = C / groups;
    for (int c = threadIdx.x; c < C; c += 256) {
        const int g0 = (c / cpg) * cpg;
        double s = 0.0, q = 0.0;
        for (int k = 0; k < cpg; ++k) {
            s += stats[((int64_t)b * C + g0 + k) * 2];
            q += stats[((int64_t)b * C + g0 + k) * 2 + 1];
        }
        const double cnt = (double)cpg * (double)HW;
        const double mean = s / cnt;
        double var = q / cnt - mean * mean;
        if (var < 0.0) var = 0.0;
        sc[c] = (float)(1.0 / sqrt(var + (double)eps)) * gamma[c];
        sh[c] = beta[c];
        mn[c] = (float)mean;
    }
    __syncthreads();
    const int c4n = C >> 2;
    for (int i = threadIdx.x; i < 64 * c4n; i += 256) {
        const int t = i / c4n, c = (i - t * c4n) * 4;
        const int p = min(p0 + t, HW - 1);
        float4 v = *reinterpret_cast<const float4*>(x + ((int64_t)b * HW + p) * C + c);
        v.x = (v.x - mn[c]) * sc[c] + sh[c];
        v.y = (v.y - mn[c + 1]) * sc[c + 1] + sh[c + 1];
        v.z = (v.z - mn[c + 2]) * sc[c + 2] + sh[c + 2];
        v.w = (v.w - mn[c + 3]) * sc[c + 3] + sh[c + 3];
        if (relu) { v.x = fmaxf(v.x, 0.f); v.y = fmaxf(v.y, 0.f); v.z = fmaxf(v.z, 0.f); v.w = fmaxf(v.w, 0.f); }
        tile[(c + 0) * 68 + t] = v.x;
        tile[(c + 1) * 68 + t] = v.y;
        tile[(c + 2) * 68 + t] = v.z;
        tile[(c + 3) * 68 + t] = v.w;
    }
    __syncthreads();
    for (int i = threadIdx.x; i < C * 16; i += 256) {
        const int c = i >> 4, t4 = (i & 15) * 4;
        if (p0 + t4 < HW)
            *reinterpret_cast<float4*>(y + ((int64_t)b * C + c) * HW + p0 + t4) = *reinterpret_cast<const float4*>(tile + c * 68 + t4);
    }
}

__global__ __launch_bounds__(256) void pos_embed_kernel(float* __restrict__ out, int H, int W, int npf, int64_t s_c,
                                                        int64_t s_p, const float* __restrict__ add_c,
                                                        float temperature, float scale) {
    const int64_t total = (int64_t)H * W * 2 * npf;
    for (int64_t idx = (int64_t)blockIdx.x * 256 + threadIdx.x; idx < total; idx += (int64_t)gridDim.x * 256) {
        const int c = (int)(idx % (2 * npf));
        const int p = (int)(idx / (2 * npf));
        const int yy = p / W, xx = p - yy * W;
        const bool is_y = c < npf;
        const int i = is_y ? c : c - npf;
        const float eps = 1e-6f;
        const float e = is_y ? ((float)(yy + 1) / ((float)H + eps) * scale) : ((float)(xx + 1) / ((float)W + eps) * scale);
        const float dim_t = powf(temperature, (float)(2 * (i / 2)) / (float)npf);
        const float a = e / dim_t;
        float v = (i & 1) ? cosf(a) : sinf(a);
        if (add_c) v += add_c[c];
        out[(int64_t)c * s_c + (int64_t)p * s_p] = v;
    }
}

__global__ __launch_bounds__(256) void transpose_kernel(const float* __restrict__ in, float* __restrict__ out, int R, int C) {
    __shared__ float tile[32][33];
    const int b = blockIdx.z;
    const int r0 = blockIdx.y * 32, c0 = blockIdx.x * 32;
    const int tx = threadIdx.x & 31, ty = threadIdx.x >> 5;
    const float* ib = in + (int64_t)b * R * C;
    float* ob = out + (int64_t)b * R * C;
    for (int k = ty; k < 32; k += 8) {
        const int r = r0 + k, c = c0 + tx;
        tile[k][tx] = (r < R && c < C) ? ib[(int64_t)r * C + c] : 0.f;
    }
    __syncthreads();
    for (int k = ty; k < 32; k += 8) {
        const int c = c0 + k, r = r0 + tx;
        if (r < R && c < C) ob[(int64_t)c * R + r] = tile[tx][k];
    }
}

__global__ __launch_bounds__(256) void nchw_to_tokens_f16_kernel(const float* __restrict__ in, unsigned short* __restrict__ out, int HW) {
    __shared__ float tile[64][65];
    const int b = blockIdx.y, p0 = blockIdx.x * 64;
    const int tid = threadIdx.x;
    const float* ib = in + (int64_t)b * 64 * HW;
    {
        const int p = tid & 63, cg = tid >> 6;
        const int pp = min(p0 + p, HW - 1);
#pragma unroll
        for (int i = 0; i < 16; ++i) tile[cg * 16 + i][p] = ib[(int64_t)(cg * 16 + i) * HW + pp];
    }
    __syncthreads();
    const int pix = tid >> 2, qd = tid & 3;
    if (p0 + pix < HW) {
        unsigned w[8];
#pragma unroll
        for (int j = 0; j < 8; ++j) {
            const float a = __builtin_amdgcn_fmed3f(tile[qd * 16 + 2 * j][pix], -65504.f, 65504.f);
            const float c = __builtin_amdgcn_fmed3f(tile[qd * 16 + 2 * j + 1][pix], -65504.f, 65504.f);
            w[j] = (unsigned)__builtin_bit_cast(unsigned short, (_Float16)a) | ((unsigned)__builtin_bit_cast(unsigned short, (_Float16)c) << 16);
        }
        uint4* dst = reinterpret_cast<uint4*>(out + ((int64_t)b * HW + p0 + pix) * 64 + qd * 16);
        dst[0] = make_uint4(w[0], w[1], w[2], w[3]);
        dst[1] = make_uint4(w[4], w[5], w[6], w[7]);
    }
}

template <int CMAX>
__global__ __launch_bounds__(256) void l2norm_nchw_kernel(const float* __restrict__ x, float* __restrict__ y, int C, int64_t hw, float eps) {
    const int b = blockIdx.y;
    const float* xb = x + (int64_t)b * C * hw;
    float* yb = y + (int64_t)b * C * hw;
    for (int64_t p = (int64_t)blockIdx.x * 256 + threadIdx.x; p < hw; p += (int64_t)gridDim.x * 256) {
        float ss = 0.f;
        float v[CMAX > 0 ? CMAX : 1];
        if constexpr (CMAX > 0) {
#pragma unroll
            for (int c = 0; c < CMAX; ++c)
                if (c < C) {
                    v[c] = xb[(int64_t)c * hw + p];
                    ss += v[c] * v[c];
                }
        } else {
            for (int c = 0; c < C; ++c) {
                const float t = xb[(int64_t)c * hw + p];
// ... 53 lines not shown
#define LN_CASE(V)                                                                                             \
    hipLaunchKernelGGL((layernorm_kernel<V>), grid, block, 0, st, x, parts, n_parts, part_stride, bias, g1, b1, \
                       l2norm, g2, b2, y, y2, rows, eps)
    switch (E) {
        case 64: LN_CASE(1); break;
        case 128: LN_CASE(2); break;
        case 256: LN_CASE(4); break;
        case 512: LN_CASE(8); break;
        default: MSM_REQUIRE(false, "msm_layernorm_f32: unsupported E=%d", E);
    }
#undef LN_CASE
    MSM_CHECK_LAUNCH("msm_layernorm_f32");
    return MSM_OK;
}

extern "C" int msm_groupnorm_stats_f32(const float* x, double* stats, int stats_cleared, int B, int HW, int C, void* stream) {
    MSM_REQUIRE(x && stats && B > 0 && HW > 0, "msm_groupnorm_stats_f32: bad arguments");
    MSM_REQUIRE(C >= 4 && C <= 256 && C % 4 == 0 && 1024 % C == 0, "msm_groupnorm_stats_f32: C=%d must be a multiple of 4 dividing 1024", C);
    MSM_REQUIRE((((uintptr_t)x) & 15) == 0, "msm_groupnorm_stats_f32: x must be 16-byte aligned");
    hipStream_t st = (hipStream_t)stream;
    if (!stats_cleared) MSM_CHECK_HIP(hipMemsetAsync(stats, 0, sizeof(double) * 2 * (size_t)B * C, st));
    const int ppb = 256;
    dim3 grid(cdiv(HW, ppb), B), block(256);
    hipLaunchKernelGGL(gn_stats_kernel, grid, block, 0, st, x, stats, HW, C, ppb);
    MSM_CHECK_LAUNCH("msm_groupnorm_stats_f32");
    return MSM_OK;
}

static int groupnorm_apply_impl(const char* who, const float* x, const double* stats, const float* gamma, const float* beta,
                                       const float* up, int uh, int uw, int64_t up_batch_stride, float* y, int B, int H, int W,
                                       int C, int groups, float eps, int relu, uint16_t* planes, void* stream, int h16 = 0) {
    MSM_REQUIRE(x && stats && gamma && beta && (y || planes), "%s: null pointer", who);
    MSM_REQUIRE(groups > 0 && C % groups == 0 && C % 4 == 0 && C <= 256, "%s: C=%d groups=%d", who, C, groups);
    MSM_REQUIRE(((((uintptr_t)x) | ((uintptr_t)y) | ((uintptr_t)up)) & 15) == 0, "%s: pointers must be 16-byte aligned", who);
    MSM_REQUIRE(!up || (uh > 0 && uw > 0), "%s: bad upsample source size", who);
    if (up_batch_stride == 0) up_batch_stride = (int64_t)uh * uw * C;
    MSM_REQUIRE(!up || (up_batch_stride >= (int64_t)uh * uw * C && up_batch_stride % 4 == 0), "%s: bad upsample batch stride", who);
    hipStream_t st = (hipStream_t)stream;
    const int64_t total = (int64_t)H * W * (C / 4);
    dim3 grid((unsigned)min((int64_t)1024, (total + 255) / 256), B), block(256);
    hipLaunchKernelGGL(gn_apply_kernel, grid, block, 0, st, x, stats, gamma, beta, up, uh, uw, up_batch_stride, y, H, W, C, groups, eps,
                       relu, planes, (int64_t)B * H * W * C, h16);
    MSM_CHECK_LAUNCH(who);
    return MSM_OK;
}

extern "C" int msm_groupnorm_apply_f32(const float* x, const double* stats, const float* gamma, const float* beta,
                                       const float* up, int uh, int uw, int64_t up_batch_stride, float* y, int B, int H, int W,
                                       int C, int groups, float eps, int relu, void* stream) {
    MSM_REQUIRE(y, "msm_groupnorm_apply_f32: null pointer");
    return groupnorm_apply_impl("msm_groupnorm_apply_f32", x, stats, gamma, beta, up, uh, uw, up_batch_stride, y, B, H, W, C, groups, eps, relu,
                                nullptr, stream);
}

extern "C" int msm_groupnorm_apply_split(const float* x, const double* stats, const float* gamma, const float* beta,
                                         const float* up, int uh, int uw, int64_t up_batch_stride, uint16_t* planes, int B, int H, int W,
                                         int C, int groups, float eps, int relu, void* stream) {
    MSM_REQUIRE(planes && (((uintptr_t)planes) & 15) == 0, "msm_groupnorm_apply_split: planes must be a 16-byte aligned pointer");
    return groupnorm_apply_impl("msm_groupnorm_apply_split", x, stats, gamma, beta, up, uh, uw, up_batch_stride, nullptr, B, H, W, C, groups, eps,
                                relu, planes, stream);
}

extern "C" int msm_groupnorm_apply_f16(const float* x, const double* stats, const float* gamma, const float* beta,
                                       const float* up, int uh, int uw, int64_t up_batch_stride, void* y_f16, int B, int H, int W,
                                       int C, int groups, float eps, int relu, void* stream) {
    MSM_REQUIRE(y_f16 && (((uintptr_t)y_f16) & 15) == 0, "msm_groupnorm_apply_f16: y must be a 16-byte aligned pointer");
    return groupnorm_apply_impl("msm_groupnorm_apply_f16", x, stats, gamma, beta, up, uh, uw, up_batch_stride, nullptr, B, H, W, C, groups, eps,
                                relu, (uint16_t*)y_f16, stream, 1);
}

extern "C" int msm_groupnorm_apply_nchw_f32(const float* x, const double* stats, const float* gamma, const float* beta, float* y,
                                            int B, int HW, int C, int groups, float eps, int relu, void* stream) {
    MSM_REQUIRE(x && stats && gamma && beta && y && x != y, "msm_groupnorm_apply_nchw_f32: null or aliased pointer");
    MSM_REQUIRE(B > 0 && HW > 0 && HW % 4 == 0, "msm_groupnorm_apply_nchw_f32: HW=%d must be a positive multiple of 4", HW);
    MSM_REQUIRE(groups > 0 && C % groups == 0 && C % 4 == 0 && C >= 4 && C <= 128, "msm_groupnorm_apply_nchw_f32: C=%d groups=%d", C, groups);
    MSM_REQUIRE(((((uintptr_t)x) | ((uintptr_t)y)) & 15) == 0, "msm_groupnorm_apply_nchw_f32: pointers must be 16-byte aligned");
    const size_t lds = sizeof(float) * ((size_t)3 * C + (size_t)C * 68);
    dim3 grid(cdiv(HW, 64), B), block(256);
    hipLaunchKernelGGL(gn_apply_nchw_kernel, grid, block, lds, (hipStream_t)stream, x, stats, gamma, beta, y, HW, C, groups, eps, relu);
    MSM_CHECK_LAUNCH("msm_groupnorm_apply_nchw_f32");
    return MSM_OK;
}

extern "C" int msm_pos_embed_sine(float* out, int H, int W, int npf, int64_t s_c, int64_t s_p, const float* add_c,
                                  float temperature, float scale, void* stream) {
    MSM_REQUIRE(out && H > 0 && W > 0 && npf > 0, "msm_pos_embed_sine: bad arguments");
    hipStream_t st = (hipStream_t)stream;
    const int64_t total = (int64_t)H * W * 2 * npf;
    dim3 grid((unsigned)min((int64_t)2048, (total + 255) / 256)), block(256);
    hipLaunchKernelGGL(pos_embed_kernel, grid, block, 0, st, out, H, W, npf, s_c, s_p, add_c, temperature, scale);
    MSM_CHECK_LAUNCH("msm_pos_embed_sine");
    return MSM_OK;
}

extern "C" int msm_transpose_f32(const float* in, float* out, int B, int R, int C, void* stream) {
    MSM_REQUIRE(in && out && B > 0 && R > 0 && C > 0, "msm_transpose_f32: bad arguments");
    hipStream_t st = (hipStream_t)stream;
    dim3 grid(cdiv(C, 32), cdiv(R, 32), B), block(256);
    hipLaunchKernelGGL(transpose_kernel, grid, block, 0, st, in, out, R, C);
    MSM_CHECK_LAUNCH("msm_transpose_f32");
    return MSM_OK;
}

extern "C" int msm_nchw_to_tokens_f16(const float* in, void* out, int B, int C, int HW, void* stream) {
    MSM_REQUIRE(in && out && B > 0 && HW > 0, "msm_nchw_to_tokens_f16: bad arguments");
    MSM_REQUIRE(C == 64, "msm_nchw_to_tokens_f16: C=%d, only 64 channels", C);
    MSM_REQUIRE((((uintptr_t)out) & 15) == 0, "msm_nchw_to_tokens_f16: out must be 16-byte aligned");
    hipLaunchKernelGGL(nchw_to_tokens_f16_kernel, dim3(cdiv(HW, 64), B), dim3(256), 0, (hipStream_t)stream, in, (unsigned short*)out, HW);
    MSM_CHECK_LAUNCH("msm_nchw_to_tokens_f16");
    return MSM_OK;
}

extern "C" int msm_l2_normalize_nchw_f32(const float* x, float* y, int B, int C, int HW, float eps, void* stream) {
    MSM_REQUIRE(x && y, "msm_l2_normalize_nchw_f32: null pointer");
    MSM_REQUIRE(B > 0 && C > 0 && HW > 0, "msm_l2_normalize_nchw_f32: bad shape");
    const int64_t hw = HW;
    dim3 grid((unsigned)max((int64_t)1, min((hw + 255) / 256, (int64_t)max(1, 8192 / B))), B), block(256);
    if (C <= 64) hipLaunchKernelGGL(l2norm_nchw_kernel<64>, grid, block, 0, (hipStream_t)stream, x, y, C, hw, eps);
    else hipLaunchKernelGGL(l2norm_nchw_kernel<0>, grid, block, 0, (hipStream_t)stream, x, y, C, hw, eps);
    MSM_CHECK_LAUNCH("msm_l2_normalize_nchw_f32");
    return MSM_OK;
}

extern "C" int msm_msda_locations(const float* offsets, const float* logits, const float* reference_points, const int64_t* spatial_shapes,
                                  float* sampling_loc, float* attn_weight, int64_t rows, int M, int L, int P, void* stream) {
    MSM_REQUIRE(offsets && logits && reference_points && spatial_shapes && sampling_loc && attn_weight, "msm_msda_locations: null pointer");
    MSM_REQUIRE(rows > 0 && M > 0 && L > 0 && P > 0, "msm_msda_locations: bad sizes");
    hipLaunchKernelGGL(msda_locations_kernel, dim3((unsigned)min((int64_t)4096, (rows * M + 255) / 256)), dim3(256), 0, (hipStream_t)stream,
                       offsets, logits, reference_points, spatial_shapes, sampling_loc, attn_weight, rows, M, L, P);
    MSM_CHECK_LAUNCH("msm_msda_locations");
    return MSM_OK;
}
```

unseenobjectswithmeanshift_amd/meta_arch.py:

```python
import inspect

import torch
import torch.nn.functional as F
from torch import nn

from . import ops
from ._plan import PlanAttributes

_ACCEPTS = {}


def _accepts(method, name):
    f = getattr(method, "__func__", method)
    key = (f, name)
    if key not in _ACCEPTS:
        _ACCEPTS[key] = name in inspect.signature(f).parameters
    return _ACCEPTS[key]


class Instances:

    def __init__(self, image_size, **fields):
        self.image_size = tuple(image_size)
        self._fields = dict(fields)
# ... 32 lines not shown
    def to(self, device):
        return Instances(self.image_size, **{k: v.to(device) for k, v in self._fields.items()})


def group_by_size(sizes):
    index = {}
    groups = []
    for i, key in enumerate(sizes):
        if key not in index:
            index[key] = len(groups)
            groups.append((key, []))
        groups[index[key]][1].append(i)
    inverse = [0] * len(sizes)
    pos = 0
    for _, members in groups:
        for i in members:
            inverse[i] = pos
            pos += 1
    return groups, inverse


def _pad_to(x, frame):
    dh, dw = frame[0] - x.shape[-2], frame[1] - x.shape[-1]
    return F.pad(x, (0, dw, 0, dh)) if dh or dw else x


class MeanShiftMaskFormerHead(PlanAttributes, nn.Module):
    _version = 2

    def __init__(self, input_shape, *, num_classes, pixel_decoder, loss_weight=1.0, ignore_value=-1,
                 transformer_predictor, transformer_in_feature="multi_scale_pixel_decoder"):
        super().__init__()
        if transformer_in_feature != "multi_scale_pixel_decoder":
            raise NotImplementedError("only TRANSFORMER_IN_FEATURE == 'multi_scale_pixel_decoder'")
        input_shape = sorted(input_shape.items(), key=lambda x: x[1].stride)
        self.in_features = [k for k, v in input_shape]
        self.ignore_value = ignore_value
        self.common_stride = 4
        self.loss_weight = loss_weight
        self.pixel_decoder = pixel_decoder
        self.predictor = transformer_predictor
        self.transformer_in_feature = transformer_in_feature
        self.num_classes = num_classes

    def _load_from_state_dict(self, state_dict, prefix, local_metadata, strict, missing_keys, unexpected_keys,
                              error_msgs):
        version = local_metadata.get("version", None)
        if version is None or version < 2:
            for k in list(state_dict.keys()):
                if k.startswith(prefix) and "sem_seg_head" in k and not k.startswith(prefix + "predictor") \
                        and not k.startswith(prefix + "pixel_decoder"):
                    state_dict[k.replace(prefix, prefix + "pixel_decoder.")] = state_dict.pop(k)
        super()._load_from_state_dict(state_dict, prefix, local_metadata, strict, missing_keys, unexpected_keys,
                                      error_msgs)

    def forward(self, features, image_height=None, image_width=None, mask=None, final_topk=0):
        return self.layers(features, image_height, image_width, mask, final_topk)

    def set_precision(self, mode):
        if mode not in ("f32", "f32_split", "bf16", "f16"):
            raise ValueError("precision must be 'f32', 'f32_split', 'bf16' or 'f16'")
        self.precision = mode
        lowp = mode in ("bf16", "f16")
        if hasattr(self.pixel_decoder, "precision"):
            self.pixel_decoder.precision = "bf16" if lowp else mode
        if hasattr(self.pixel_decoder, "lp_operands"):
            self.pixel_decoder.lp_operands = "f16" if mode == "f16" else "bf16"
        low = "bf16" if lowp else "f32"
        self.predictor.mask_step_dtype = "f32_split" if mode == "f32_split" else (mode if lowp else "f32")
        if hasattr(self.predictor, "tails_dtype"):
            self.predictor.tails_dtype = mode if lowp else "f32"
        if hasattr(self.predictor, "attention_dtype"):
            self.predictor.attention_dtype = low
        if hasattr(self.predictor, "attention_keys"):
            self.predictor.attention_keys = "f16" if mode == "f16" else "bf16"
        if hasattr(self.predictor, "kv_split"):
            self.predictor.kv_split = mode == "f32_split"
        return self

    def layers(self, features, image_height=None, image_width=None, mask=None, final_topk=0):
        kw = {}
        if getattr(self.predictor, "folded_mask_features", False) and _accepts(self.pixel_decoder.forward_features, "folded"):
            kw["folded"] = True
        mask_features, _, multi_scale_features = self.pixel_decoder.forward_features(features, **kw)
        if final_topk and _accepts(self.predictor.forward, "final_topk"):
            predictions = self.predictor(multi_scale_features, mask_features, mask, final_topk=final_topk)
        else:
            predictions = self.predictor(multi_scale_features, mask_features, mask)
        return predictions, None


class PretrainedMeanShiftMaskFormerHead(MeanShiftMaskFormerHead):
    """meanshift_former_head.py:145-275: identical glue for the UCN (RGB-D) configuration; the reference
    calls exit() for any TRANSFORMER_IN_FEATURE other than "multi_scale_pixel_decoder" (:258-274)."""


class MeanShiftMaskFormer(PlanAttributes, nn.Module):

    def __init__(self, *, backbone, sem_seg_head, num_queries, test_topk_per_image=20, size_divisibility=32,
                 instance_on=True, pixel_mean=None, pixel_std=None):
        super().__init__()
        if (pixel_mean is None) != (pixel_std is None):
            raise ValueError("pixel_mean and pixel_std go together")
        if pixel_mean is not None:
            self.register_buffer("pixel_mean", torch.tensor(pixel_mean, dtype=torch.float32).view(-1, 1, 1), False)
            self.register_buffer("pixel_std", torch.tensor(pixel_std, dtype=torch.float32).view(-1, 1, 1), False)
        else:
            self.pixel_mean = self.pixel_std = None
        self.backbone = backbone
        self.sem_seg_head = sem_seg_head
        self.num_queries = num_queries
        self.test_topk_per_image = test_topk_per_image
        self.size_divisibility = size_divisibility
        self.instance_on = instance_on

    def _select(self, features, padded_size):
        k = int(self.test_topk_per_image) if getattr(self, "topk_before_masks", True) else 0
        if k and _accepts(self.sem_seg_head.forward, "final_topk"):
            outputs, _ = self.sem_seg_head(features, padded_size[0], padded_size[1], final_topk=k)
        else:
            outputs, _ = self.sem_seg_head(features, padded_size[0], padded_size[1])
        if "topk" in outputs:
            cls_scores, classes, qidx = outputs["topk"]
            B, K = qidx.shape
            key = (B, K, str(qidx.device))
            if getattr(self, "_iota", (None,))[0] != key:
                self._iota = (key, torch.arange(K, device=qidx.device, dtype=torch.int32)[None].expand(B, -1).contiguous())
            local = self._iota[1]
        else:
            cls_scores, classes, qidx = ops.topk_class_scores(outputs["pred_logits"], self.test_topk_per_image)
            local = qidx
        return outputs["pred_masks"], local, cls_scores, classes, qidx

    @torch.no_grad()
    def inference(self, features, image_size, padded_size=None, output_size=None):
        padded_size = tuple(padded_size or image_size)
        low, local, cls_scores, classes, qidx = self._select(features, padded_size)
        masks, scores, boxes = ops.instance_postprocess(low, local, image_size, class_scores=cls_scores,
                                                        padded_size=padded_size, output_size=output_size)
        return scores, classes, masks, boxes, qidx

    def _image_features(self, inputs):
        return self.backbone(inputs["image"], inputs["depth"]) if "depth" in inputs else self.backbone(inputs["image"])

    @torch.no_grad()
    def inference_images(self, inputs, image_size, padded_size=None, output_size=None):
        if self.backbone is None:
            raise RuntimeError("inference_images needs a backbone")
        return self.inference(self._image_features(inputs), image_size, padded_size, output_size)

    def _forward_images(self, batched_inputs, keys, normalise):
        first = batched_inputs[0]
        div = max(int(self.size_divisibility), 1)
        if first[keys[0]].dim() == 4:
            batch = {k: first[k] for k in keys}
            n = batch[keys[0]].shape[0]
            H, W = (int(v) for v in batch[keys[0]].shape[-2:])
            sizes = [((H, W), (int(first.get("height", H)), int(first.get("width", W))))] * n
            samples = None
        else:
            samples = batched_inputs
            sizes = []
            for x in samples:
                H, W = (int(v) for v in x[keys[0]].shape[-2:])
                sizes.append(((H, W), (int(x.get("height", H)), int(x.get("width", W)))))
        frame = (-(-max(s[0][0] for s in sizes) // div) * div, -(-max(s[0][1] for s in sizes) // div) * div)
# ... 172 lines not shown
```

unseenobjectswithmeanshift_amd/modeling.py:

```python
import math

import torch
from torch import nn

from . import ops
from ._plan import PlanAttributes, TensorList, version_key

KAPPA = 30


class ShapeSpec:

    def __init__(self, channels=None, height=None, width=None, stride=None):
        self.channels, self.height, self.width, self.stride = channels, height, width, stride


class PositionEmbeddingSine(nn.Module):
    def __init__(self, num_pos_feats=64, temperature=10000, normalize=False, scale=None):
        super().__init__()
        if scale is not None and normalize is False:
            raise ValueError("normalize should be True if scale is passed")
        if not normalize:
            raise NotImplementedError("the hot path only uses normalize=True (DEC:415, MSD:241)")
        self.num_pos_feats = num_pos_feats
        self.temperature = temperature
        self.normalize = normalize
        self.scale = 2 * math.pi if scale is None else scale

    def forward(self, x, mask=None):
        if mask is not None:
            raise NotImplementedError("padding masks are not used by the MSMFormer configs")
        B, _, H, W = x.shape
        pe = ops.pos_embed_sine(H, W, self.num_pos_feats, x.device, temperature=float(self.temperature),
                                scale=float(self.scale))
        return pe[None].expand(B, -1, -1, -1)


def hypersphere_attention(q, k, v, attn_mask=None, dropout_p=0.0, kappa=KAPPA):
    if dropout_p > 0.0:
        raise NotImplementedError("inference only")
    Bh, Nt, E = q.shape
    if E != 32:
        raise RuntimeError("head_dim must be 32")
    masked = row_any = None
    if attn_mask is not None:
        masked = (attn_mask == float("-inf")).to(torch.uint8).contiguous()
        row_any = torch.ones((Bh, Nt), device=q.device, dtype=torch.int32)
    return ops.hypersphere_attention(q.contiguous(), k.contiguous(), v.contiguous(), 1, masked=masked,
                                     row_any=row_any, kappa=float(kappa))


class FoldedMaskFeatures:

    def __init__(self, act, weight, bias, materialize):
        self.act, self.weight, self.bias = act, weight, bias
        self._materialize = materialize
        self._tensor = None

    @property
    def shape(self):
        B, _, H, W = self.act.shape
        return torch.Size((B, self.weight.shape[0], H, W))

    @property
    def device(self):
        return self.act.device

    def tensor(self):
        if self._tensor is None:
            self._tensor = self._materialize()
        return self._tensor


class ConvFoldedMaskFeatures:

    def __init__(self, x, weight, bias, materialize):
        self.x, self.weight, self.bias = x, weight, bias
        self._materialize = materialize
        self._tensor = None

    @property
    def shape(self):
        B, _, H, W = self.x.shape
        return torch.Size((B, self.weight.shape[0], H, W))

    @property
    def device(self):
        return self.x.device

    def tensor(self):
        if self._tensor is None:
            self._tensor = self._materialize()
        return self._tensor


class MeanShiftAttention(nn.Module):

    def __init__(self, embed_dim, num_heads=1, dropout=0., bias=True, add_bias_kv=False, add_zero_attn=False,
                 kdim=None, vdim=None, batch_first=False, device=None, dtype=None):
        super().__init__()
        self.embed_dim = embed_dim
        self.num_heads = num_heads
        self.batch_first = False
        self.in_proj_weight = nn.Parameter(torch.empty(3 * embed_dim, embed_dim))
        self.in_proj_bias = nn.Parameter(torch.zeros(3 * embed_dim))
        self.out_proj = nn.Linear(embed_dim, embed_dim)
        nn.init.xavier_uniform_(self.in_proj_weight)
        nn.init.constant_(self.out_proj.bias, 0.)

    def attend(self, tgt, memory_k, memory_v, *, query_pos=None, key_pos=None, masked=None, row_any=None,
               kv=None):
        E = self.embed_dim
        w, b = self.in_proj_weight, self.in_proj_bias
        q = ops.gemm(tgt, w[:E], b[:E], a2=query_pos)
        if kv is None:
            k = ops.gemm(memory_k, w[E:2 * E], b[E:2 * E], a2=key_pos)
            v = ops.gemm(memory_v, w[2 * E:], b[2 * E:])
        else:
            k, v = kv
        o = ops.hypersphere_attention(q, k, v, self.num_heads, masked=masked, row_any=row_any, kappa=float(KAPPA))
        return ops.gemm(o, self.out_proj.weight, self.out_proj.bias)

    def project_kv(self, memory, pos):
        E = self.embed_dim
        w, b = self.in_proj_weight, self.in_proj_bias
        return ops.gemm(memory, w[E:2 * E], b[E:2 * E], a2=pos), ops.gemm(memory, w[2 * E:], b[2 * E:])

    @torch.no_grad()
    def forward(self, query, key, value, key_padding_mask=None, need_weights=True, attn_mask=None):
        if key_padding_mask is not None:
            raise NotImplementedError("key_padding_mask is unused by the MSMFormer decoder (DEC:622)")
        L, N, E = query.shape
        S = key.shape[0]
        q = query.transpose(0, 1).contiguous()
        k = key.transpose(0, 1).contiguous()
        v = value.transpose(0, 1).contiguous()
        masked = row_any = None
        if attn_mask is not None:
# ... 161 lines not shown
                a = layer.meanshift_attn
                wk, wv = a.in_proj_weight[E:2 * E].double(), a.in_proj_weight[2 * E:].double()
                bk, bv = a.in_proj_bias[E:2 * E].double(), a.in_proj_bias[2 * E:].double()
                lvl = self.level_embed.weight[l].double()
                if isinstance(self.input_proj[l], nn.Conv2d):
                    wp = self.input_proj[l].weight.view(E, -1).double()
                    off = self.input_proj[l].bias.double() + lvl
                else:
                    wp = torch.eye(E, dtype=torch.float64, device=device)
                    off = lvl
                pos = self._pos_tokens(h, w, device).double()
                ws.append(torch.cat([wk @ wp, wv @ wp], 0).float().contiguous())
                pg, E2 = pos.view(h, w, E), E // 2
                if (self.separable_kv_constants and h > 1 and w > 1 and h * w >= sep_min and torch.equal(pg[:, :1, :E2].expand(h, w, E2), pg[..., :E2])
                        and torch.equal(pg[:1, :, E2:].expand(h, w, E - E2), pg[..., E2:])):
                    row = torch.cat([pg[:, 0, :E2] @ wk[:, :E2].t() + (off @ wk.t() + bk), (off @ wv.t() + bv).expand(h, -1)], 1)
                    col = torch.cat([pg[0, :, E2:] @ wk[:, E2:].t(), torch.zeros(w, E, dtype=torch.float64, device=device)], 1)
                    cs.append((torch.cat([row, col], 0).float().contiguous(), w))
                else:
                    kc = (pos + off) @ wk.t() + bk
                    vc = (off @ wv.t() + bv).expand(h * w, -1)
                    cs.append((torch.cat([kc, vc], 1).float().contiguous(), 0))
            self._kv_cache[skey] = (ws, cs)
        return self._kv_cache[skey]

    def _heads(self, d, mask_features, target_size, want_mask, want_cls):
        cls = ops.gemm(d, self.class_embed.weight, self.class_embed.bias) if want_cls else None
        e = self.mask_embed(d)
        mask, attn, row_any = ops.mask_logits(e, mask_features, want_mask=want_mask, target_size=target_size,
                                              sparse=self.sparse_taps, packed_bf16=self._packed_mf,
                                              packed_split=getattr(self, "_packed_mf_split", None))
        return cls, mask, attn, row_any

    def _packed_tails(self):
        E = self.query_feat.weight.shape[1]
        groups = {
            "cross_q": [l.meanshift_attn.in_proj_weight[:E] for l in self.transformer_cross_attention_layers],
            "cross_o": [l.meanshift_attn.out_proj.weight for l in self.transformer_cross_attention_layers],
            "self_in": [l.self_attn.in_proj_weight for l in self.transformer_self_attention_layers],
            "self_o": [l.self_attn.out_proj.weight for l in self.transformer_self_attention_layers],
            "ffn1": [l.linear1.weight for l in self.transformer_ffn_layers],
            "ffn2": [l.linear2.weight for l in self.transformer_ffn_layers],
            "mlp": [l.weight for l in self.mask_embed.layers],
        }
        kernel_of = {"cross_q": "heads", "mlp": "heads", "cross_o": "post_cross", "self_in": "post_cross", "self_o": "post_self", "ffn1": "post_self",
                     "ffn2": "post_self"}
        key = (self.tails_dtype, str(self.tails_hl)) + tuple((p.data_ptr(), p._version) for ws in groups.values() for p in ws)
        if self._tails_cache is None or self._tails_cache[0] != key:
            self._tails_cache = (key, {k: [self._tails_pack(kernel_of[k])(w.contiguous()) for w in ws] for k, ws in groups.items()})
        return self._tails_cache[1]

    def _tails_hl_for(self, kernel):
        return self.tails_dtype == "bf16" and (self.tails_hl is True or (isinstance(self.tails_hl, (tuple, list, set, frozenset)) and kernel in self.tails_hl))

    def _tails_pack(self, kernel="heads"):
        hl = self._tails_hl_for(kernel)
        try:
            return {"f32": ops.dec_pack_weight, "bf16": ops.dec_pack_weight_bf16x2 if hl else ops.dec_pack_weight_bf16,
                    "f16": ops.dec_pack_weight_f16}[self.tails_dtype]
        except KeyError:
            raise ValueError("tails_dtype must be 'f32', 'bf16' or 'f16'") from None

    def _folded_head(self, fm):
        l3 = self.mask_embed.layers[-1]
        params = (l3.weight, l3.bias, fm.weight) + ((fm.bias,) if fm.bias is not None else ())
        pack = self._tails_pack()
        key = (self.tails_dtype, str(self.tails_hl)) + tuple((p.data_ptr(), p._version) for p in params)
        if self._fold_cache is None or self._fold_cache[0] != key:
            wm = fm.weight.detach().double().reshape(fm.weight.shape[0], -1)
            bm = fm.bias.detach().double() if fm.bias is not None else torch.zeros(wm.shape[0], dtype=torch.float64, device=wm.device)
            w3, b3 = l3.weight.detach().double(), l3.bias.detach().double()
            n = wm.shape[1]
            w = torch.zeros_like(w3)
            b = torch.zeros_like(b3)
            w[:n] = wm.t() @ w3
            w[n] = bm @ w3
            b[:n] = wm.t() @ b3
            b[n] = bm @ b3
            self._fold_cache = (key, pack(w.float().contiguous()), b.float().contiguous(), n)
        return self._fold_cache[1:]

    @staticmethod
    def _poolable_sizes(act, sizes):
        Hm, Wm = int(act.shape[2]), int(act.shape[3])
        out = []
        for (th, tw) in sizes:
            if (int(th), int(tw)) not in out and Hm % th == 0 and Wm % tw == 0 and Hm // th == Wm // tw and Hm // th in (2, 4, 8):
                out.append((int(th), int(tw)))
        return out

    def _keys_f16(self):
        return self.attention_dtype == "bf16" and self.attention_keys == "f16" and 2 * self.query_feat.weight.shape[1] == 512

    def _kv_one(self, x, w, cc):
        c, cw = cc
        if x.shape[1] == 64 and w.shape[0] in (256, 512):
            if self.attention_dtype == "bf16":
                return ops.kv_project_multi([x], [w], [c], out_dtype=torch.bfloat16, cmat_widths=[cw],
                                            keys_f16=self._keys_f16())[0]
            if self.kv_split:
                return ops.kv_project_multi([x], [w], [c], split=True, cmat_widths=[cw])[0]
        return ops.kv_project(x, w, c, cw)

    def _uniform_constants(self, kv_c, jobs):
        cs = [kv_c[i] for i in jobs]
        if len({cw > 0 for _, cw in cs}) <= 1:
            return cs
        out = []
        for i, (c, cw) in zip(jobs, cs):
            if cw > 0:
                key = ("dense", i, c.data_ptr(), tuple(c.shape))
                if key not in self._kv_cache:
                    self._kv_cache[key] = ops.dense_kv_constant(c, cw)
                c, cw = self._kv_cache[key], 0
            out.append((c, cw))
        return out

    def _fused_kv_plan(self, xs, sizes, kv_w, kv_c):
        if not (self.fused_kv_attention and self.fused_tails and self.attention_dtype == "bf16"):
            return None
        E = self.query_feat.weight.shape[1]
        H = self.num_heads
        cache = self._kv_cache.setdefault(("fkv", tuple(sizes), str(xs[0].device)), {})
        layers, xh = [], {}
        for i in range(self.num_layers):
            l = i % self.num_feature_levels
            h, w = sizes[l]
            c, cw = kv_c[i]
            if not (cw == w and w % 16 == 0 and h * w >= int(self.fused_kv_min_keys) and xs[l].shape[1] == 64 and tuple(kv_w[i].shape) == (2 * E, 64) and E == H * 32
                    and h * w * 128 < (1 << 32)):
                layers.append(None)
                continue
            if i not in cache:
                cache[i] = (ops.attn_pack_kv_weights(kv_w[i], H), c, c[h:, E:].t().contiguous())
            layers.append(cache[i])
            if l not in xh:
                xh[l] = ops.tokens_f16(xs[l])
        return {"layers": layers, "x": xh} if xh else None

    def _forward_fused(self, xs, sizes, kv_w, kv_c, mask_features, out, qpos, kv_all=None, final_topk=0, fkv=None):
        E = self.query_feat.weight.shape[1]
        L = self.num_layers
        full = self.aux_outputs
        H = self.num_heads
        pk = self._packed_tails()
        mlp = [(pk["mlp"][j], l.bias) for j, l in enumerate(self.mask_embed.layers)]
        ncol = None
        pooled = {}
        ra0 = None
        ra_all, fuse_masks = None, False
        fm_params = None
        if isinstance(mask_features, FoldedMaskFeatures):
            fm_params = [t for t in (mask_features.weight, mask_features.bias) if t is not None]
            wf, bf, ncol = self._folded_head(mask_features)
            mlp[-1] = (wf, bf)
            mask_features = mask_features.act
            if self.pooled_attention_masks and (not full or self.pooled_attention_masks == "always") and ncol == 64 and mask_features.shape[1] == 64:
                want_sizes = self._poolable_sizes(mask_features, sizes)
                if want_sizes and L > 0:
                    fuse_masks = bool(self.fused_head_masks) and self.tails_dtype in ("bf16", "f16") and not self._tails_hl_for("heads") and not full \
                        and self.lp_pooled_masks != "x3"
                    Bq, Qn = int(out.shape[0]), int(out.shape[1])
                    outs, flags = ops.pool_mask_taps(mask_features, want_sizes, zero_rows=Qn * (L + 1 if fuse_masks else 1))
                    ra_all = flags.view(-1)[:Bq * Qn * (L + 1 if fuse_masks else 1)].view(-1, Bq, Qn)
                    ra0 = ra_all[0]
                    pooled = dict(zip(want_sizes, outs))
        dn = self.decoder_norm
        pred_cls, pred_mask = [], []
        topk_out = []
        cf = None
        if isinstance(mask_features, ConvFoldedMaskFeatures):
            wkey = ("cfw", str(mask_features.device)) + version_key([mask_features.weight, mask_features.bias])
            wc = getattr(self, "_conv_fold_cache", None)
            if wc is None or wc[0] != wkey:
                self._conv_fold_cache = wc = (wkey, ops.mask_conv_fold_weight(mask_features.weight, mask_features.bias))
            cf = (fkv["x"][0], wc[1])

        def predict_conv_folded(d, e, ra, i_next):
            last = i_next == L
            x16, wf = cf
            if not last:
                attn, row_any = ops.mask_conv3x3_folded(x16, ops.gemm(e, wf), sizes[0], bits=True, row_any=ra)
                pred_cls.append(None)
                pred_mask.append(None)
                return attn, row_any
            cls = ops.gemm(d, self.class_embed.weight, self.class_embed.bias)
            if 0 < final_topk < e.shape[1]:
                *topk, sel = ops.topk_class_scores(cls, int(final_topk), gather=e, gather_cols=e.shape[2])
                topk_out.append(tuple(topk))
                e = sel
            pred_cls.append(cls)
            pred_mask.append(ops.mask_conv3x3_folded(x16, ops.gemm(e, wf), sizes[0], bits=False))
            return None, None

        def predict(d, e, ra, i_next):
            if cf is not None:
                return predict_conv_folded(d, e, ra, i_next)
            last = i_next == L
            want = full or last
            cls = ops.gemm(d, self.class_embed.weight, self.class_embed.bias) if want else None
            tgt = None if (last and not full) else sizes[i_next % self.num_feature_levels]
            emb, qb = (e, None) if ncol is None else (e[..., :ncol], e[..., ncol])
            if last and not full and ncol is not None and 0 < final_topk < e.shape[1] and cls is not None:
                *topk, sel = ops.topk_class_scores(cls, int(final_topk), gather=e, gather_cols=ncol + 4)
                topk = tuple(topk)
                m = ops.mask_logits(sel[..., :ncol], mask_features, want_mask=True, target_size=None, qbias=sel[..., ncol])[0]
                pred_cls.append(cls)
                pred_mask.append(m)
                topk_out.append(topk)
                return None, None
            if tgt is not None and tuple(tgt) in pooled:
                as_bits = fkv is not None and i_next < L and fkv["layers"][i_next] is not None
                attn, row_any = ops.attn_mask_pooled(emb, pooled[tuple(tgt)], qbias=qb, row_any=ra, bits=as_bits,
                                                          f16=self.lp_pooled_masks if self.mask_step_dtype in ("bf16", "f16") else False)
                m = None
                if want:
                    m = ops.mask_logits(emb, mask_features, want_mask=True, target_size=None, packed_bf16=self._packed_mf, qbias=qb,
                                        packed_split=getattr(self, "_packed_mf_split", None))[0]
                pred_cls.append(cls)
                pred_mask.append(m)
                return attn, row_any
            m, attn, row_any = ops.mask_logits(emb, mask_features, want_mask=want, target_size=tgt, sparse=self.sparse_taps,
                                               row_any=ra,
                                               packed_bf16=self._packed_mf, qbias=qb, packed_split=getattr(self, "_packed_mf_split", None))
            pred_cls.append(cls)
            pred_mask.append(m)
            return attn, row_any

        def next_query(i):
            if i >= L:
                return dict(wq=None, bq=None, query_pos=None)
            return dict(wq=pk["cross_q"][i], bq=self.transformer_cross_attention_layers[i].meanshift_attn.in_proj_bias[:E],
                        query_pos=qpos)

        if not full and L > 0 and fm_params is not None:
            if getattr(self, "_heads0_params", None) is None:
                self._heads0_params = TensorList(self.parameters)
            hkey = (tuple(out.shape), str(out.device), self.tails_dtype, str(self.tails_hl)) + version_key(self._heads0_params()) + version_key(fm_params)
            hc = getattr(self, "_heads0_cache", None)
            if hc is None or hc[0] != hkey:
                _, d, e, q, _ = ops.dec_heads(out, dn.weight, dn.bias, mlp, want_out=False, want_d=False, zero_row_any=True, **next_query(0))
                self._heads0_cache = hc = (hkey, d, e, q)
            _, d, e, q = hc
            ra = ra0
        else:
            _, d, e, q, ra = ops.dec_heads(out, dn.weight, dn.bias, mlp, want_out=False, want_d=full or L == 0,
                                           zero_row_any=True, **next_query(0))
        attn, row_any = predict(d, e, ra, 0)
        pf_on = bool(self.weight_prefetch) and out.is_cuda and (self.weight_prefetch == "always" or self.tails_dtype in ("bf16", "f16"))
# ... 503 lines not shown
                if C == 64 and all(m[0].weight.shape[1] % 256 == 0 for m in self.input_proj) else None
            self._front = (key, wpk, gnp, stream, small, wp.shape[0], hm, wlp)
        return self._front[1:]

    def _encode(self, features):
        C = self.conv_dim
        levels = [features[f].float().contiguous() for f in self.transformer_in_features[::-1]]
        B = levels[0].shape[0]
        shapes = [(int(x.shape[2]), int(x.shape[3])) for x in levels]
        dev = levels[0].device
        ss, starts, lvl_pos = self._geometry(shapes, dev)
        S_tok = sum(h * w for h, w in shapes)
        layers = self.transformer.encoder.layers
        gns = [m[1] for m in self.input_proj]
        front = (self.fused_encoder and self.fused_front and C == 64 and len(levels) <= 4 and S_tok >= 86
                 and all(x.shape[1] % 128 == 0 and (x.shape[2] * x.shape[3]) % 4 == 0 for x in levels)
                 and all(g.num_groups == gns[0].num_groups and g.eps == gns[0].eps for g in gns))
        value = proj = None
        fpn_stats = (None, None)
        if front:
            wpk, gnp, pstream, psmall, pw, phm, wlp = self._packed_front(dev)
            src = torch.empty((B, S_tok, C), device=dev, dtype=torch.float32)
            stats = torch.zeros((len(levels) + 2, B, C, 2), device=dev, dtype=torch.float64)
            fpn_stats = (stats[len(levels)], stats[len(levels) + 1])
            if self.precision == "bf16" and self.lp_input_proj == "deep" and wlp is not None and B * S_tok >= 16384:
                ops.conv1x1_in_multi(levels, wlp, [m[0].bias for m in self.input_proj], src, stats[:len(levels)], stats_cleared=True, lp="wide")
            else:
                ops.conv1x1_in_multi(levels, wpk, [m[0].bias for m in self.input_proj], src, stats[:len(levels)], stats_cleared=True)
            a0 = layers[0].self_attn
            bounds = [0]
            for h, w in shapes:
                bounds.append(bounds[-1] + h * w)
            fuse0 = self._use_fused_msda(dev)
            if self._use_hm() and phm is not None and self.lp_prologue:
                src, value, proj = ops.encoder_prologue_hm(src, stats[:len(levels)], gnp, bounds, phm[0], phm[1], lvl_pos,
                                                           groups=gns[0].num_groups, eps=gns[0].eps)
            else:
                src, value, proj = ops.encoder_prologue(src, stats[:len(levels)], gnp, bounds, pstream, psmall[:64] if fuse0 else psmall, lvl_pos,
                                                        0 if fuse0 else pw, groups=gns[0].num_groups, eps=gns[0].eps, value_heads=a0.n_heads,
                                                        bf16_hm=self._use_hm())
        else:
            toks = []
            for idx, x in enumerate(levels):
                conv, gn = self.input_proj[idx][0], self.input_proj[idx][1]
                t = ops.conv1x1_nchw_to_tokens(x, conv.weight.view(C, -1), conv.bias)
                toks.append(ops.groupnorm_tokens(t, gn.weight, gn.bias, shapes[idx][0], shapes[idx][1], groups=gn.num_groups, eps=gn.eps))
            src = torch.cat(toks, 1).contiguous()
        if self.fused_encoder and C == 64:
            packed = self._packed_encoder(dev)
            fuse = self._use_fused_msda(dev)
            if value is None:
                a0 = layers[0].self_attn
                value = ops.value_to_head_major(ops.gemm(src, a0.value_proj.weight, a0.value_proj.bias), a0.n_heads)
                if not fuse:
                    w, b = self._packed[2]
                    proj = ops.gemm(src, w, b, a2=lvl_pos)
            if self._use_hm():
                if value.dtype != torch.float16:
                    value = ops.to_f16(value if value.dim() == 4 else ops.value_to_head_major(value, 8))
                    proj = ops.proj_to_head_major_records(proj)
                for l, layer in enumerate(layers):
                    attn = ops.ms_deform_attn_encoder_lp(value, ss, starts, proj, layer.self_attn.n_points)
                    stream, small, d_ffn, _ = packed[l]
                    src, value, proj = ops.encoder_block_hm(attn, src, stream, small, d_ffn, pos=lvl_pos, want_next=l + 1 < len(layers),
                                                            eps=layer.norm1.eps, ffn_f16=self.lp_operands == "f16")
                return src, shapes, fpn_stats
            for l, layer in enumerate(layers):
                if fuse:
                    attn = ops.ms_deform_attn_encoder_fused(value, ss, starts, src, lvl_pos, *self._packed[3][l], layer.self_attn.n_points)
                else:
                    attn = ops.ms_deform_attn_encoder(value, ss, starts, proj, layer.self_attn.n_heads, layer.self_attn.n_points)
                stream, small, d_ffn, pw = packed[l]
                if fuse:
                    pw = 0
                block = {"f32": ops.encoder_block, "f32_split": ops.encoder_block_split, "bf16": ops.encoder_block_lp}[self.precision]
                src, value, proj = block(attn, src, stream, small, d_ffn, pw, pos=lvl_pos, tokens_per_image=S_tok,
                                                     want_next=l + 1 < len(layers), eps=layer.norm1.eps,
                                                     value_heads=layers[l + 1].self_attn.n_heads if l + 1 < len(layers) else 0)
        else:
            for layer in layers:
                src = layer.forward_tokens(src, lvl_pos, ss, starts)
        return src, shapes, fpn_stats

    def _fpn_mask_features(self, features, up_tok, up_hw, fpn_stats, folded=False):
        C = self.conv_dim
        B = up_tok.shape[0]
        x = features[self.in_features[0]].float().contiguous()
        H, W = int(x.shape[2]), int(x.shape[3])
        split3 = C == 64 and self.precision == "f32_split"
        half_map = C == 64 and self.precision == "bf16" and self.lp_conv3x3 and self.lp_operands == "f16" and self.fpn_half_map
        if C == 64 and x.shape[1] % 128 == 0 and x.shape[1] <= 384 and (H * W) % 4 == 0 and B * H * W >= 32 * 1024:
            lp = self._lp_input_proj([x.shape[1]])
            lat, lat_stats = ops.conv1x1_in(x, self._w_lateral(lp), None, stats=fpn_stats[0], stats_cleared=fpn_stats[0] is not None, lp=lp)
            y = ops.groupnorm_tokens(lat, self.adapter_1.norm.weight, self.adapter_1.norm.bias, H, W, groups=32,
                                     up=up_tok, up_hw=up_hw, eps=self.adapter_1.norm.eps, stats=lat_stats, stats_ready=True,
                                     split_planes=split3, out_f16=half_map)
        else:
            lat = ops.conv1x1_nchw_to_tokens(x, self.adapter_1.weight.view(C, -1), None)
            y = ops.groupnorm_tokens(lat, self.adapter_1.norm.weight, self.adapter_1.norm.bias, H, W, groups=32,
                                     up=up_tok, up_hw=up_hw, eps=self.adapter_1.norm.eps, stats=fpn_stats[0], split_planes=split3,
                                     out_f16=half_map)
        y_stats = None
        if C == 64:
            y, y_stats = ops.conv3x3_c64(y, self._w3(), H, W, stats=fpn_stats[1], stats_cleared=fpn_stats[1] is not None,
                                         bf16=(self.lp_operands == "f16" and "f16" or True) if (self.precision == "bf16" and self.lp_conv3x3) else False,
                                         split=split3)
        else:
            y = ops.conv3x3_tokens(y, self._w3(), H, W)
        wm = self.mask_features.weight.view(self.mask_dim, C)
        if C == 64 and self.mask_dim in (256, 512) and (H * W) % 4 == 0 and (B <= 64 or folded):
            gn = (y_stats, self.layer_1.norm.weight, self.layer_1.norm.bias, 32, self.layer_1.norm.eps)
            if B <= 64:
                literal = lambda: ops.tokens_proj_nchw(y, wm, self.mask_features.bias, gn=gn, relu=True).view(B, self.mask_dim, H, W)
            else:
                literal = lambda: ops.conv1x1_tokens_to_nchw(
                    ops.groupnorm_tokens(y, self.layer_1.norm.weight, self.layer_1.norm.bias, H, W, groups=32, relu=True,
                                         eps=self.layer_1.norm.eps), wm, self.mask_features.bias).view(B, self.mask_dim, H, W)
            if folded:
                act = ops.groupnorm_nchw(y, y_stats, self.layer_1.norm.weight, self.layer_1.norm.bias, groups=32,
                                         eps=self.layer_1.norm.eps, relu=True).view(B, C, H, W)
                return FoldedMaskFeatures(act, wm, self.mask_features.bias, literal)
            mask_features = literal()
        else:
            y = ops.groupnorm_tokens(y, self.layer_1.norm.weight, self.layer_1.norm.bias, H, W, groups=32, relu=True,
                                     eps=self.layer_1.norm.eps)
            mask_features = ops.conv1x1_tokens_to_nchw(y, wm, self.mask_features.bias).view(B, self.mask_dim, H, W)
        return mask_features

    @torch.no_grad()
    def forward_features(self, features, folded=False):
        C = self.conv_dim
        src, shapes, fpn_stats = self._encode(features)
        B = src.shape[0]
        out, o = [], 0
        for (h, w) in shapes:
            out.append(src[:, o:o + h * w].view(B, h, w, C).permute(0, 3, 1, 2))
            o += h * w
        up_tok = src[:, o - shapes[-1][0] * shapes[-1][1]:]
        mask_features = self._fpn_mask_features(features, up_tok, shapes[-1], fpn_stats, folded)
        return mask_features, out[0], out[:self.maskformer_num_feature_levels]
```

unseenobjectswithmeanshift_amd/ops.py:

```python
import ctypes

import torch

from ._lib import check, lib
from .packing import (MASK_CONV_K, MASK_CONV_LD, PROJ_REC_FLOATS, dense_kv_constant, mask_conv_fold_weight, pack_conv_in_weight,
                      pack_conv_in_weight_lp, pack_encoder_block, pack_encoder_block_hm, pack_encoder_block_hm_small,
                      pack_encoder_block_lp, pack_encoder_block_split, pack_encoder_prologue, pack_encoder_prologue_hm,
                      pack_msda_proj_lp, proj_records_to_columns, proj_to_head_major_records)

KAPPA = 30.0


_raw_stream = getattr(torch._C, "_cuda_getCurrentRawStream", None)
_cur_device = getattr(torch._C, "_cuda_getDevice", None)


def _stream():
    if _raw_stream is not None and _cur_device is not None:
        return ctypes.c_void_p(_raw_stream(_cur_device()))
    return ctypes.c_void_p(torch.cuda.current_stream().cuda_stream)


def _p(t):
    return ctypes.c_void_p(0 if t is None else t.data_ptr())
# ... 172 lines not shown
    else:
        _c(t, "t", torch.float16 if half_in else torch.float32)
        B, HW, C = t.shape
    _c(w_tap_major, "w"), _c(stats, "stats", torch.float64)
    if C != 64 or tuple(w_tap_major.shape) != (64, 576) or HW != H * W:
        raise RuntimeError("conv3x3_c64 needs a (B, H*W, 64) map and a (64, 576) tap-major weight")
    out = torch.empty((B, HW, C), device=t.device, dtype=torch.float32)
    if stats is None:
        stats = torch.empty((B, 64, 2), device=t.device, dtype=torch.float64)
        stats_cleared = False
    elif tuple(stats.shape) != (B, 64, 2):
        raise RuntimeError("stats must be (B, 64, 2) float64")
    name = "msm_conv3x3_c64_split" if split else "msm_conv3x3_c64_f16h" if half_in else ("msm_conv3x3_c64_f16" if bf16 == "f16" else "msm_conv3x3_c64_bf16" if bf16 else "msm_conv3x3_c64_f32")
    rc = getattr(lib(), name)(_p(t), _p(w_tap_major), _p(out), _p(stats), 1 if stats_cleared else 0, B, H, W, _stream())
    check(rc, name)
    return out, stats


def conv3x3_tokens_to_nchw(t, w_tap_major, bias, H, W, bf16=False):
    _c(t, "t"), _c(w_tap_major, "w"), _c(bias, "bias")
    B, HW, Cin = t.shape
    Cout = w_tap_major.shape[0]
    out = torch.empty((B, Cout, HW), device=t.device, dtype=torch.float32)
    if Cin == 64 and Cout % 64 == 0 and Cout <= 1024 and W % 4 == 0 and HW == H * W:
        name = "msm_conv3x3_c64_nchw_f16" if bf16 == "f16" else "msm_conv3x3_c64_nchw_bf16" if bf16 else "msm_conv3x3_c64_nchw_f32"
        rc = getattr(lib(), name)(_p(t), _p(w_tap_major), _p(bias), _p(out), B, H, W, Cout, _stream())
        check(rc, name)
        return out
    rc = lib().msm_gemm_f32(_p(t), None, _p(w_tap_major), _p(bias), _p(out), HW, Cout, 9 * Cin, B,
                            Cin, 1, HW * Cin, 0, 0, 1, HW, Cout * HW, 0,
                            2, H, W, Cin, 1 if bias is not None else 0, 0, 1, _stream())
    check(rc, "msm_gemm_f32(conv3x3 -> nchw)")
    return out


def layernorm(x, g1, b1, *, parts=None, bias=None, l2norm=False, g2=None, b2=None, eps=1e-5):
    _c(x, "x"), _c(parts, "parts"), _c(bias, "bias"), _c(g1, "g1"), _c(b1, "b1"), _c(g2, "g2"), _c(b2, "b2")
    ref = x if x is not None else parts[0]
    E = ref.shape[-1]
    rows = ref.numel() // E
    y = torch.empty_like(ref)
    y2 = torch.empty_like(ref) if g2 is not None else None
    n_parts = 0 if parts is None else parts.shape[0]
    rc = lib().msm_layernorm_f32(_p(x), _p(parts), n_parts, rows * E, _p(bias), _p(g1), _p(b1),
                                 1 if l2norm else 0, _p(g2), _p(b2), _p(y), _p(y2), rows, E, eps, _stream())
    check(rc, "msm_layernorm_f32")
    return (y, y2) if g2 is not None else y


def groupnorm_tokens(x, gamma, beta, H, W, groups=32, *, up=None, up_hw=None, relu=False, eps=1e-5, stats=None, stats_ready=False,
                     split_planes=False, out_f16=False):
    if split_planes and out_f16:
        raise RuntimeError("groupnorm_tokens: split_planes and out_f16 are different output forms")
    _c(x, "x"), _c(gamma, "gamma"), _c(beta, "beta"), _chk(up, "up")
    B, HW, C = x.shape
    if stats_ready:
        _c(stats, "stats", torch.float64)
        if stats is None or tuple(stats.shape) != (B, C, 2):
            raise RuntimeError("stats_ready needs stats (B, C, 2) float64")
    else:
        stats = groupnorm_stats(x, stats)
    y = torch.empty((3,) + tuple(x.shape), device=x.device, dtype=torch.bfloat16) if split_planes else \
        torch.empty(x.shape, device=x.device, dtype=torch.float16) if out_f16 else torch.empty_like(x)
    uh, uw = (0, 0) if up is None else up_hw
    usb = 0
    if up is not None:
        if tuple(up.shape) != (B, uh * uw, C) or up.stride(2) != 1 or up.stride(1) != C or (B > 1 and up.stride(0) < uh * uw * C):
            raise RuntimeError("up must be (B, uh*uw, C) with strides (>= uh*uw*C, C, 1)")
        usb = up.stride(0) if B > 1 else 0
    name = "msm_groupnorm_apply_split" if split_planes else "msm_groupnorm_apply_f16" if out_f16 else "msm_groupnorm_apply_f32"
    rc = getattr(lib(), name)(_p(x), _p(stats), _p(gamma), _p(beta), _p(up), uh, uw, usb, _p(y), B, H, W, C, groups, eps, 1 if relu else 0, _stream())
    check(rc, name)
    return y


def groupnorm_nchw(x, stats, gamma, beta, *, groups=32, eps=1e-5, relu=False):
    _c(x, "x"), _c(stats, "stats", torch.float64), _c(gamma, "gamma"), _c(beta, "beta")
    B, HW, C = x.shape
    y = torch.empty((B, C, HW), device=x.device, dtype=torch.float32)
    rc = lib().msm_groupnorm_apply_nchw_f32(_p(x), _p(stats), _p(gamma), _p(beta), _p(y), B, HW, C, int(groups), float(eps),
                                            1 if relu else 0, _stream())
    check(rc, "msm_groupnorm_apply_nchw_f32")
    return y


def groupnorm_stats(x, stats=None):
    _c(x, "x"), _c(stats, "stats", torch.float64)
    B, HW, C = x.shape
    cleared = stats is not None
    if stats is None:
        stats = torch.empty((B, C, 2), device=x.device, dtype=torch.float64)
    elif tuple(stats.shape) != (B, C, 2):
        raise RuntimeError("stats must be (B, C, 2) float64")
    check(lib().msm_groupnorm_stats_f32(_p(x), _p(stats), 1 if cleared else 0, B, HW, C, _stream()), "msm_groupnorm_stats_f32")
    return stats


def tokens_proj_nchw(x, w, bias=None, *, gn=None, relu=False):
    _c(x, "x"), _c(w, "w"), _c(bias, "bias")
    B, HW, C = x.shape
    N = w.shape[0]
    stats = gamma = beta = None
    groups, eps = 1, 0.0
    if gn is not None:
        stats, gamma, beta, groups, eps = gn
        _c(stats, "stats", torch.float64), _c(gamma, "gamma"), _c(beta, "beta")
    out = torch.empty((B, N, HW), device=x.device, dtype=torch.float32)
    rc = lib().msm_tokens_proj_nchw_f32(_p(x), _p(w), _p(bias), _p(stats), _p(gamma), _p(beta), int(groups), float(eps),
                                        1 if relu else 0, _p(out), B, C, HW, N, _stream())
    check(rc, "msm_tokens_proj_nchw_f32")
    return out


def pos_embed_sine(H, W, num_pos_feats, device, *, layout="nchw", add_c=None, temperature=10000.0,
                   scale=6.283185307179586):
    C = 2 * num_pos_feats
    _c(add_c, "add_c")
    if layout == "nchw":
        out = torch.empty((C, H, W), device=device, dtype=torch.float32)
        s_c, s_p = H * W, 1
    else:
        out = torch.empty((H * W, C), device=device, dtype=torch.float32)
        s_c, s_p = 1, C
    rc = lib().msm_pos_embed_sine(_p(out), H, W, num_pos_feats, s_c, s_p, _p(add_c), temperature, scale, _stream())
    check(rc, "msm_pos_embed_sine")
    return out


def transpose_last2(x):
    _c(x, "x")
    B, R, C = x.shape
    out = torch.empty((B, C, R), device=x.device, dtype=torch.float32)
    check(lib().msm_transpose_f32(_p(x), _p(out), B, R, C, _stream()), "msm_transpose_f32")
    return out


def l2_normalize_nchw(x, eps=1e-12):
    _c(x, "x")
    B, C, H, W = x.shape
    y = torch.empty_like(x)
    check(lib().msm_l2_normalize_nchw_f32(_p(x), _p(y), B, C, H * W, float(eps), _stream()), "msm_l2_normalize_nchw_f32")
    return y


def msda_locations(offsets, logits, reference_points, spatial_shapes):
    _c(offsets, "offsets"), _c(logits, "logits"), _c(reference_points, "reference_points"), _c(spatial_shapes, "spatial_shapes", torch.int64)
    N, Lq, M, L, P, _ = offsets.shape
    if tuple(logits.shape) != (N, Lq, M, L * P) or tuple(reference_points.shape) != (N, Lq, L, 2):
        raise RuntimeError("msda_locations: logits must be (N,Lq,M,L*P) and reference_points (N,Lq,L,2)")
    loc = torch.empty_like(offsets)
    attn = torch.empty((N, Lq, M, L, P), device=offsets.device, dtype=torch.float32)
    check(lib().msm_msda_locations(_p(offsets), _p(logits), _p(reference_points), _p(spatial_shapes), _p(loc), _p(attn), N * Lq, M, L, P,
                                   _stream()), "msm_msda_locations")
    return loc, attn


def pack_mask_features_bf16(mask_features, f16=False):
    _c(mask_features, "mask_features")
    B, C, H, W = mask_features.shape
    out = torch.empty((B, C // 4, H * W, 4), device=mask_features.device, dtype=torch.float16 if f16 else torch.int16)
    name = "msm_pack_mask_features_f16" if f16 else "msm_pack_mask_features_bf16"
    rc = getattr(lib(), name)(_p(mask_features), _p(out), B, C, H * W, _stream())
    check(rc, name)
    return out


# ... 1158 lines not shown
```

Measured before the change: 3852 images/sec.

## Fuse groupnorm NCHW apply with mask-tap pooling and add short-query mask kernel

Adds a kernel that applies groupnorm, writes the NCHW activation, computes the pooled mask taps for each requested level and zeroes the row-any flags in one pass. The decoder then reuses these pooled outputs instead of launching a separate pool_mask_taps pass that re-reads the activation. Separately, the mask-logits kernel is templated on the number of query blocks so that small-Q writes can use a 2-block variant with less LDS. The cost is extra plumbing between the pixel decoder and the predictor, with a fallback when the handed-off plan does not match.

```diff
diff --git a/include/msm_hip.h b/include/msm_hip.h
--- a/include/msm_hip.h
+++ b/include/msm_hip.h
@@ -13,7 +13,7 @@
 #define MSM_E_WORKSPACE (-3)
 
 const char* msm_last_error_string(void);
-#define MSM_ABI_VERSION 28
+#define MSM_ABI_VERSION 29
 int msm_abi_version(void);
 
 #define MSM_OPT_AUTO (-1)
@@ -39,6 +39,7 @@
     MSM_OPT_CONV3_WIDE,
     MSM_OPT_DEC_TILE32,
     MSM_OPT_POST_RESIZE_DIRECT,
+    MSM_OPT_GN_POOL,
     MSM_OPT_COUNT
 };
 int msm_set_option(int key, int value);
@@ -71,6 +72,9 @@
 
 int msm_groupnorm_apply_nchw_f32(const float* x, const double* stats, const float* gamma, const float* beta, float* y,
                                  int B, int HW, int C, int groups, float eps, int relu, void* stream);
+int msm_groupnorm_nchw_pool_f32(const float* x, const double* stats, const float* gamma, const float* beta, float* y, int B,
+                                int H, int W, int C, int groups, float eps, int relu, int n_levels, const int32_t* th,
+                                const int32_t* tw, float* const* out, int32_t* zero_buf, int64_t zero_count, void* stream);
 
 int msm_pos_embed_sine(float* out, int H, int W, int npf, int64_t s_c, int64_t s_p,
                        const float* add_c, float temperature, float scale, void* stream);
diff --git a/unseenobjectswithmeanshift_amd/_lib.py b/unseenobjectswithmeanshift_amd/_lib.py
--- a/unseenobjectswithmeanshift_amd/_lib.py
+++ b/unseenobjectswithmeanshift_amd/_lib.py
@@ -7,7 +7,7 @@
 HEADER_PATH = os.path.join(os.path.dirname(_HERE), "include", "msm_hip.h")
 
 _lib = None
-ABI_VERSION = 28
+ABI_VERSION = 29
 
 c_f = ctypes.c_void_p
 c_p = ctypes.c_void_p
@@ -29,6 +29,7 @@
     "msm_groupnorm_apply_split": (c_i, [c_f, c_p, c_f, c_f, c_f, c_i, c_i, c_l, c_f, c_i, c_i, c_i, c_i, c_i, c_fl, c_i, c_p]),
     "msm_groupnorm_apply_f16": (c_i, [c_f, c_p, c_f, c_f, c_f, c_i, c_i, c_l, c_p, c_i, c_i, c_i, c_i, c_i, c_fl, c_i, c_p]),
     "msm_groupnorm_apply_nchw_f32": (c_i, [c_f, c_p, c_f, c_f, c_f, c_i, c_i, c_i, c_i, c_fl, c_i, c_p]),
+    "msm_groupnorm_nchw_pool_f32": (c_i, [c_f, c_p, c_f, c_f, c_f, c_i, c_i, c_i, c_i, c_i, c_fl, c_i, c_i, c_p, c_p, c_p, c_p, c_l, c_p]),
     "msm_pos_embed_sine": (c_i, [c_f, c_i, c_i, c_i, c_l, c_l, c_f, c_fl, c_fl, c_p]),
     "msm_transpose_f32": (c_i, [c_f, c_f, c_i, c_i, c_i, c_p]),
     "msm_l2_normalize_nchw_f32": (c_i, [c_f, c_f, c_i, c_i, c_i, c_fl, c_p]),
@@ -196,7 +197,7 @@
 
 OPTIONS = ("MASK_NC", "MASKB_TARGET", "GEMM_TILE", "GEMM_SHALLOW", "ATTN_TARGET", "ATTN_KERNEL", "ATTN_QK_MAX", "ATTN_QKCFG",
            "CONVIN_NT", "POST_GENERIC", "ENC_NO_COOP", "MSDA_GENERIC", "MS_CHUNK", "MS_NO_PERSISTENT", "ATTN_FUSED_KV", "KV_PIPE", "MASK_KERNEL",
-           "MS_SPLIT_KERNEL", "CONV3_WIDE", "DEC_TILE32", "POST_RESIZE_DIRECT")
+           "MS_SPLIT_KERNEL", "CONV3_WIDE", "DEC_TILE32", "POST_RESIZE_DIRECT", "GN_POOL")
 OPT_AUTO = -1
 
 
diff --git a/unseenobjectswithmeanshift_amd/csrc/mask_logits.hip b/unseenobjectswithmeanshift_amd/csrc/mask_logits.hip
--- a/unseenobjectswithmeanshift_amd/csrc/mask_logits.hip
+++ b/unseenobjectswithmeanshift_amd/csrc/mask_logits.hip
@@ -9,6 +9,7 @@
 
 constexpr int QB = 7;
 constexpr int QCH = QB * 16;
+constexpr int QBS = 2;
 #ifndef MSM_MASK_KU
 #define MSM_MASK_KU 4
 #endif
@@ -70,14 +71,14 @@
     }
 };
 
-template <int NC>
-__device__ __forceinline__ float acc_val(const f32x4 (&acc)[QB][2 * NC], int m, int row, int j) {
+template <int NC, int NQ>
+__device__ __forceinline__ float acc_val(const f32x4 (&acc)[NQ][2 * NC], int m, int row, int j) {
     if constexpr (NC == 2) return acc[m][row * 2 + (j & 1)][j >> 1];
     else return acc[m][row][j];
 }
 
-template <int POOL, bool WRITE, int NC, bool DO_WRITE = true, bool DO_ATTN = true, bool R4 = false>
-__device__ __forceinline__ void mask_tile_epilogue(const f32x4 (&acc)[QB][2 * NC], float* __restrict__ mask_out,
+template <int POOL, bool WRITE, int NC, bool DO_WRITE = true, bool DO_ATTN = true, bool R4 = false, int NQ = QB>
+__device__ __forceinline__ void mask_tile_epilogue(const f32x4 (&acc)[NQ][2 * NC], float* __restrict__ mask_out,
                                                    uint8_t* __restrict__ attn_out, int* __restrict__ any_flags, int b, int Q,
                                                    int q0, int H, int W, int th, int tw, int ytop, int ybot, int c0, int lj, int lq) {
     using PM = PixMap<POOL, NC>;
@@ -87,8 +88,8 @@
     const int xb = c0 + NP * lq;
     if constexpr (WRITE && DO_WRITE) {
 #pragma unroll
-        for (int m = 0; m < QB; ++m) {
-            const bool rem = R4 && m == QB - 1;
+        for (int m = 0; m < NQ; ++m) {
+            const bool rem = R4 && m == NQ - 1;
             const int pg = rem ? (ql >> 2) : lq;
             const int xb = c0 + NP * pg;
             const bool vec = !PM::PERM && xb + NP <= W && (W & 3) == 0;
@@ -121,7 +122,7 @@
         const int HW = H * W;
         const bool vec = xb + NP <= W && (W & 3) == 0;
 #pragma unroll
-        for (int m = 0; m < QB; ++m) {
+        for (int m = 0; m < NQ; ++m) {
             const int q = q0 + m * 16 + ql;
             if (q >= Q) continue;
             uint8_t* o = attn_out + ((int64_t)b * Q + q) * HW;
@@ -161,7 +162,7 @@
         static_assert(PM::PERM || NP >= POOL, "a lane must hold whole taps");
         const bool vec = NT == 4 ? ((tw & 3) == 0 && tx0 + 4 <= tw) : (NT == 2 ? ((tw & 1) == 0 && tx0 + 2 <= tw) : (tx0 < tw));
 #pragma unroll
-        for (int m = 0; m < QB; ++m) {
+        for (int m = 0; m < NQ; ++m) {
             uint32_t w = 0;
 #pragma unroll
             for (int t = 0; t < NT; ++t) {
@@ -193,11 +194,11 @@
     }
 }
 
-template <int POOL, bool WRITE, int NC>
+template <int POOL, bool WRITE, int NC, int NQ = QB>
 struct MaskEpiConst {
-    unsigned aoff[QB];
-    unsigned moff[QB];
-    unsigned anyv[QB];
+    unsigned aoff[NQ];
+    unsigned moff[NQ];
+    unsigned anyv[NQ];
     __amdgpu_buffer_rsrc_t arsrc, mrsrc;
     bool attn_fast, write_fast;
 };
@@ -215,8 +216,8 @@
                    (uint64_t)(unsigned)__builtin_amdgcn_readfirstlane((int)(unsigned)u));
 }
 
-template <int POOL, bool WRITE, int NC>
-__device__ __forceinline__ void mask_epi_init(MaskEpiConst<POOL, WRITE, NC>& k, float* mask_out, uint8_t* attn_out, int b, int Q, int q0,
+template <int POOL, bool WRITE, int NC, int NQ>
+__device__ __forceinline__ void mask_epi_init(MaskEpiConst<POOL, WRITE, NC, NQ>& k, float* mask_out, uint8_t* attn_out, int b, int Q, int q0,
                                               int H, int W, int th, int tw, int lj, int lq, bool r4 = false) {
     using PM = PixMap<POOL, NC>;
     constexpr int NP = 4 * NC;
@@ -224,8 +225,8 @@
     const int TT = POOL == 1 ? HW : th * tw;
     constexpr int NT = PM::PERM ? 1 : (POOL == 1 ? NP : (NP / (POOL > 0 ? POOL : 1) > 0 ? NP / (POOL > 0 ? POOL : 1) : 1));
 #pragma unroll
-    for (int m = 0; m < QB; ++m) {
-        const bool rem = r4 && m == QB - 1;
+    for (int m = 0; m < NQ; ++m) {
+        const bool rem = r4 && m == NQ - 1;
         const int pgl = rem ? (lj >> 2) : lq;
         const int q = rem ? q0 + m * 16 + (lj & 3) : q0 + m * 16 + lj;
         const int lane_key = POOL == 1 ? NP * pgl : (PM::PERM ? (pgl >> 1) : (NP * pgl) / (POOL > 0 ? POOL : 1));
@@ -245,8 +246,8 @@
 
 typedef unsigned int u32x4 __attribute__((ext_vector_type(4)));
 
-template <int POOL, bool WRITE, int NC, bool DO_WRITE, bool DO_ATTN, bool R4_PARTIAL = false>
-__device__ __forceinline__ void mask_tile_epilogue_fast(const f32x4 (&acc)[QB][2 * NC], MaskEpiConst<POOL, WRITE, NC>& k, int H, int W, int tw,
+template <int POOL, bool WRITE, int NC, bool DO_WRITE, bool DO_ATTN, bool R4_PARTIAL = false, int NQ = QB>
+__device__ __forceinline__ void mask_tile_epilogue_fast(const f32x4 (&acc)[NQ][2 * NC], MaskEpiConst<POOL, WRITE, NC, NQ>& k, int H, int W, int tw,
                                                         int ytop, int ybot, int c0) {
     using PM = PixMap<POOL, NC>;
     constexpr int NP = 4 * NC;
@@ -258,7 +259,7 @@
             if (y < 0 || y >= H) continue;
             const unsigned soff = (unsigned)(y * W + c0) * 4u;
 #pragma unroll
-            for (int m = 0; m < QB; ++m)
+            for (int m = 0; m < NQ; ++m)
 #pragma unroll
                 for (int j = 0; j < NP; j += 4)
                     __builtin_amdgcn_raw_buffer_store_b128(u32x4{__float_as_uint(acc_val<NC>(acc, m, row, j)), __float_as_uint(acc_val<NC>(acc, m, row, j + 1)),
@@ -275,7 +276,7 @@
             if (y < 0 || y >= H) continue;
             const unsigned soff = (unsigned)(y * W + c0);
 #pragma unroll
-            for (int m = 0; m < QB; ++m)
+            for (int m = 0; m < NQ; ++m)
 #pragma unroll
                 for (int j0 = 0; j0 < NP; j0 += 4) {
                     unsigned w = 0;
@@ -293,7 +294,7 @@
         static_assert(PM::PERM || NP >= POOL, "a lane must hold whole taps");
         const unsigned soff = (unsigned)((ytop / POOL) * tw + c0 / POOL);
 #pragma unroll
-        for (int m = 0; m < QB; ++m) {
+        for (int m = 0; m < NQ; ++m) {
             unsigned w = 0;
 #pragma unroll
             for (int t = 0; t < NT; ++t) {
@@ -301,7 +302,7 @@
                 float s = add1(add1(acc_val<NC>(acc, m, 0, jl), acc_val<NC>(acc, m, 0, jl + 1)),
                                add1(acc_val<NC>(acc, m, 1, jl), acc_val<NC>(acc, m, 1, jl + 1)));
                 if constexpr (R4_PARTIAL) {
-                    if (m == QB - 1) {
+                    if (m == NQ - 1) {
                         s = sum_lane_rows(s);
                     }
                 }
@@ -330,16 +331,16 @@
     }
 }
 
-template <int POOL, bool WRITE, int NC>
-__device__ __forceinline__ void mask_epi_flush(const MaskEpiConst<POOL, WRITE, NC>& k, int* __restrict__ any_flags, int lj, bool r4 = false) {
+template <int POOL, bool WRITE, int NC, int NQ>
+__device__ __forceinline__ void mask_epi_flush(const MaskEpiConst<POOL, WRITE, NC, NQ>& k, int* __restrict__ any_flags, int lj, bool r4 = false) {
     if constexpr (POOL != 0) {
 #pragma unroll
-        for (int m = 0; m < QB; ++m)
-            if (k.anyv[m] != 0u && k.aoff[m] != 0xF0000000u) any_flags[m * 16 + ((r4 && m == QB - 1) ? (lj & 3) : lj)] = 1;
-    }
-}
-
-template <int POOL, bool WRITE, int NC, int D, bool R4 = false>
+        for (int m = 0; m < NQ; ++m)
+            if (k.anyv[m] != 0u && k.aoff[m] != 0xF0000000u) any_flags[m * 16 + ((r4 && m == NQ - 1) ? (lj & 3) : lj)] = 1;
+    }
+}
+
+template <int POOL, bool WRITE, int NC, int D, bool R4 = false, int NQ = QB>
 __global__ __launch_bounds__(MW * 64) void mask_logits_kernel(const float* __restrict__ emb, const float* __restrict__ feat,
                                                           float* __restrict__ mask_out, uint8_t* __restrict__ attn_out,
                                                           int32_t* __restrict__ row_any, int Q, int C, int H, int W,
@@ -348,6 +349,7 @@
                                                           const float* __restrict__ qbias, int64_t qbias_ld) {
     extern __shared__ __attribute__((aligned(16))) float Es[];
     constexpr int TW = 16 * NC;
+    constexpr int QCH = NQ * 16;
     constexpr int NA = 2 * NC;
     const int SE = C + 2;
     const int b = blockIdx.z, qc = blockIdx.y;
@@ -436,18 +438,18 @@
     __syncthreads();
     MASK_TS(1)
 
-    constexpr int NB4 = NC == 1 ? QB : 1;
+    constexpr int NB4 = NC == 1 ? NQ : 1;
     f32x4 bias4[NB4];
     if constexpr (NC == 1) {
 #pragma unroll
-        for (int m = 0; m < QB; ++m) {
+        for (int m = 0; m < NQ; ++m) {
             float q_b = qb[m * 16 + lj];
-            if (R4 && m == QB - 1) q_b = lq == 0 ? qb[m * 16 + (lj & 3)] : 0.f;
+            if (R4 && m == NQ - 1) q_b = lq == 0 ? qb[m * 16 + (lj & 3)] : 0.f;
             bias4[m] = f32x4{q_b, q_b, q_b, q_b};
         }
     }
     static_assert(!R4 || NC == 1, "the 4-query block exists for 2 x 16 tiles only");
-    MaskEpiConst<POOL, WRITE, NC> epi;
+    MaskEpiConst<POOL, WRITE, NC, NQ> epi;
     mask_epi_init<POOL, WRITE, NC>(epi, mask_out, attn_out, b, Q, q0, H, W, th, tw, lj, lq, R4);
 
     const int G = C / (4 * KU);
@@ -463,15 +465,15 @@
         unsigned nvoff_top, nvoff_bot;
         tile_voffs(tile_of(min(it + 1, my_tiles - 1)), nvoff_top, nvoff_bot);
 
-        f32x4 acc[QB][NA];
+        f32x4 acc[NQ][NA];
         auto compute_group = [&](auto first, const Cols<NC>(&t_)[KU], const Cols<NC>(&bt)[KU], int kbase) {
 #pragma unroll
             for (int u = 0; u < KU; ++u) {
                 const float* er = &Es[lj * SE + kbase + u * 4 + lq];
 #pragma unroll
-                for (int m = 0; m < QB; ++m) {
+                for (int m = 0; m < NQ; ++m) {
                     if constexpr (R4) {
-                        if (m == QB - 1) {
+                        if (m == NQ - 1) {
                             const float a4 = Es[(m * 16 + (lj & 3)) * SE + kbase + u * 4 + lq];
                             if (decltype(first)::value && u == 0) {
                                 acc[m][0] = __builtin_amdgcn_mfma_f32_4x4x1f32(t_[u].v[0], a4, bias4[m], 0, 0, 0);
@@ -523,7 +525,7 @@
         MASK_TS(2 + 3 * it)
 #ifdef MSM_MASK_TS
         {
-            float dep = acc[QB - 1][NA - 1][3];
+            float dep = acc[NQ - 1][NA - 1][3];
             asm volatile("v_mov_b32 %0, %0" : "+v"(dep));
             MASK_TS(3 + 3 * it)
         }
@@ -536,9 +538,9 @@
                 for (int row = 0; row < 2; ++row)
 #pragma unroll
                     for (int r = 0; r < 4; ++r) {
-                        float v = acc[QB - 1][row][r];
+                        float v = acc[NQ - 1][row][r];
                         v = sum_lane_rows(v);
-                        acc[QB - 1][row][r] = v;
+                        acc[NQ - 1][row][r] = v;
                     }
             }
         }
@@ -926,15 +928,17 @@
     if (mask_out) nc = 1;
     const int ctiles = cdiv(W, 16 * nc);
     const int ntiles = n_rowpairs * ctiles;
+    const bool wr = mask_out != nullptr;
+    const bool shortq = wr && pool == 0 && Q <= 16 * QBS && opt(MSM_OPT_MASK_KERNEL) != 7;
+    const int qch = shortq ? 16 * QBS : QCH;
     int wg_per = cdiv(ntiles, MW);
-    const size_t lds = sizeof(float) * ((size_t)QCH * (C + 2) + 2 * QCH);
+    const size_t lds = sizeof(float) * ((size_t)qch * (C + 2) + 2 * qch);
     const int target = cdiv(256, B * qchunks);
     if (wg_per > target) wg_per = max(target, 1);
     dim3 grid(wg_per, qchunks, B), block(MW * 64);
     typedef void (*kern_t)(const float*, const float*, float*, uint8_t*, int32_t*, int, int, int, int, int, int, int, int, int, int, int, int64_t,
                            const float*, int64_t);
     kern_t kern;
-    const bool wr = mask_out != nullptr;
     const bool r4 = nc == 1 && Q == 100 && W % 16 == 0 && (int64_t)Q * H * W * 4 < 0xF0000000ll && opt(MSM_OPT_MASK_KERNEL) != 5 &&
                     (pool == 0 || pool == 2 || pool == 4 || pool == 8);
 #define MASK_PICK(P)                                                                                                   \
@@ -949,6 +953,7 @@
         default: kern = MASK_PICK(8); break;
     }
 #undef MASK_PICK
+    if (shortq) kern = (C / (4 * KU)) % 4 == 0 ? (kern_t)mask_logits_kernel<0, true, 1, 4, false, QBS> : (kern_t)mask_logits_kernel<0, true, 1, 2, false, QBS>;
     MSM_CHECK_HIP((hipError_t)ensure_dynamic_lds((const void*)kern, lds));
     hipLaunchKernelGGL(kern, grid, block, lds, st, mask_embed, mask_feat, mask_out, attn_out, row_any, Q, C, H, W, th, tw,
                        ypar, n_rowpairs, rp_step, rp_first, (int)((int64_t)C * H * W * 4), embed_ld, qbias, qbias_ld);
diff --git a/unseenobjectswithmeanshift_amd/csrc/norm.hip b/unseenobjectswithmeanshift_amd/csrc/norm.hip
--- a/unseenobjectswithmeanshift_amd/csrc/norm.hip
+++ b/unseenobjectswithmeanshift_amd/csrc/norm.hip
@@ -234,6 +234,96 @@
     }
 }
 
+constexpr int GP_C = 64, GP_TH = 8, GP_TW = 16, GP_S = GP_TH * GP_TW + 4, GP_MAXL = 4, GP_T = 512;
+struct GnPoolLevels {
+    int n;
+    int lg[GP_MAXL], th[GP_MAXL], tw[GP_MAXL];
+    float* out[GP_MAXL];
+};
+__global__ __launch_bounds__(GP_T) void gn_apply_nchw_pool_kernel(const float* __restrict__ x, const double* __restrict__ stats,
+                                                                 const float* __restrict__ gamma, const float* __restrict__ beta,
+                                                                 float* __restrict__ y, GnPoolLevels lv, int H, int W, int groups, float eps,
+                                                                 int relu, int32_t* __restrict__ zero_buf, int64_t zero_count) {
+    constexpr int C = GP_C;
+    __shared__ float sc[C], sh[C], mn[C];
+    __shared__ __attribute__((aligned(16))) float tile[C * GP_S];
+    const int tid = threadIdx.x;
+    const int b = blockIdx.z, r0 = blockIdx.y * GP_TH, c0 = blockIdx.x * GP_TW;
+    const int HW = H * W;
+    if (zero_buf) {
+        const int64_t nthreads = (int64_t)gridDim.x * gridDim.y * gridDim.z * GP_T;
+        for (int64_t i = (((int64_t)blockIdx.z * gridDim.y + blockIdx.y) * gridDim.x + blockIdx.x) * GP_T + tid; i < zero_count; i += nthreads)
+            zero_buf[i] = 0;
+    }
+    const int cpg = C / groups;
+    if (tid < C) {
+        const int c = tid, g0 = (c / cpg) * cpg;
+        double s = 0.0, q = 0.0;
+        for (int k = 0; k < cpg; ++k) {
+            s += stats[((int64_t)b * C + g0 + k) * 2];
+            q += stats[((int64_t)b * C + g0 + k) * 2 + 1];
+        }
+        const double cnt = (double)cpg * (double)HW;
+        const double mean = s / cnt;
+        double var = q / cnt - mean * mean;
+        if (var < 0.0) var = 0.0;
+        sc[c] = (float)(1.0 / sqrt(var + (double)eps)) * gamma[c];
+        sh[c] = beta[c];
+        mn[c] = (float)mean;
+    }
+    __syncthreads();
+    constexpr int NI = GP_TH * GP_TW * (C / 4) / GP_T;
+    float4 v_[NI];
+#pragma unroll
+    for (int k = 0; k < NI; ++k) {
+        const int i = tid + k * GP_T;
+        const int t = i >> 4, c = (i & 15) * 4;
+        const int p = min(r0 + (t >> 4), H - 1) * W + min(c0 + (t & 15), W - 1);
+        v_[k] = *reinterpret_cast<const float4*>(x + ((int64_t)b * HW + p) * C + c);
+    }
+#pragma unroll
+    for (int k = 0; k < NI; ++k) {
+        const int i = tid + k * GP_T;
+        const int t = i >> 4, c = (i & 15) * 4;
+        float4 v = v_[k];
+        v.x = (v.x - mn[c]) * sc[c] + sh[c];
+        v.y = (v.y - mn[c + 1]) * sc[c + 1] + sh[c + 1];
+        v.z = (v.z - mn[c + 2]) * sc[c + 2] + sh[c + 2];
+        v.w = (v.w - mn[c + 3]) * sc[c + 3] + sh[c + 3];
+        if (relu) { v.x = fmaxf(v.x, 0.f); v.y = fmaxf(v.y, 0.f); v.z = fmaxf(v.z, 0.f); v.w = fmaxf(v.w, 0.f); }
+        tile[(c + 0) * GP_S + t] = v.x;
+        tile[(c + 1) * GP_S + t] = v.y;
+        tile[(c + 2) * GP_S + t] = v.z;
+        tile[(c + 3) * GP_S + t] = v.w;
+    }
+    __syncthreads();
+    for (int i = tid; i < C * GP_TH * (GP_TW / 4); i += GP_T) {
+        const int c = i >> 5, ry = (i >> 2) & 7, x4 = (i & 3) * 4;
+        if (r0 + ry < H && c0 + x4 < W)
+            *reinterpret_cast<float4*>(y + (((int64_t)b * C + c) * H + r0 + ry) * W + c0 + x4) =
+                *reinterpret_cast<const float4*>(tile + c * GP_S + ry * GP_TW + x4);
+    }
+    for (int l = 0; l < lv.n; ++l) {
+        const int lg = lv.lg[l], pp = 1 << lg, th = lv.th[l], tw = lv.tw[l];
+        const int lx = 4 - lg;
+        const int nt = (GP_TH >> lg) << lx;
+        float* ob = lv.out[l] + (int64_t)b * th * tw * C;
+        for (int i = tid; i < nt * (C / 4); i += GP_T) {
+            const int tt = i >> 4, c4 = (i & 15) * 4;
+            const int jy = tt >> lx, jx = tt & ((1 << lx) - 1);
+            const int ty = (r0 >> lg) + jy, tx = (c0 >> lg) + jx;
+            if (ty >= th || tx >= tw) continue;
+            const float* q = tile + c4 * GP_S + ((jy << lg) + pp / 2 - 1) * GP_TW + (jx << lg) + pp / 2 - 1;
+            float4 r;
+            r.x = 0.25f * ((q[0] + q[1]) + (q[GP_TW] + q[GP_TW + 1]));
+            r.y = 0.25f * ((q[GP_S] + q[GP_S + 1]) + (q[GP_S + GP_TW] + q[GP_S + GP_TW + 1]));
+            r.z = 0.25f * ((q[2 * GP_S] + q[2 * GP_S + 1]) + (q[2 * GP_S + GP_TW] + q[2 * GP_S + GP_TW + 1]));
+            r.w = 0.25f * ((q[3 * GP_S] + q[3 * GP_S + 1]) + (q[3 * GP_S + GP_TW] + q[3 * GP_S + GP_TW + 1]));
+            *reinterpret_cast<float4*>(ob + ((int64_t)ty * tw + tx) * C + c4) = r;
+        }
+    }
+}
+
 __global__ __launch_bounds__(256) void pos_embed_kernel(float* __restrict__ out, int H, int W, int npf, int64_t s_c,
                                                         int64_t s_p, const float* __restrict__ add_c,
                                                         float temperature, float scale) {
@@ -453,6 +543,41 @@
     return MSM_OK;
 }
 
+extern "C" int msm_groupnorm_nchw_pool_f32(const float* x, const double* stats, const float* gamma, const float* beta, float* y, int B,
+                                          int H, int W, int C, int groups, float eps, int relu, int n_levels, const int32_t* th,
+                                          const int32_t* tw, float* const* out, int32_t* zero_buf, int64_t zero_count, void* stream) {
+    MSM_REQUIRE(x && stats && gamma && beta && y && x != y, "msm_groupnorm_nchw_pool_f32: null or aliased pointer");
+    MSM_REQUIRE(B > 0 && H > 1 && W > 1 && W % 4 == 0, "msm_groupnorm_nchw_pool_f32: %dx%d: W must be a multiple of 4", H, W);
+    MSM_REQUIRE(C == GP_C && groups > 0 && C % groups == 0, "msm_groupnorm_nchw_pool_f32: C=%d groups=%d (the 64-channel activation)", C, groups);
+    MSM_REQUIRE(((((uintptr_t)x) | ((uintptr_t)y)) & 15) == 0, "msm_groupnorm_nchw_pool_f32: pointers must be 16-byte aligned");
+    MSM_REQUIRE(!zero_buf || zero_count > 0, "msm_groupnorm_nchw_pool_f32: zero_buf needs a positive count");
+    MSM_REQUIRE(th && tw && out && n_levels >= 1 && n_levels <= GP_MAXL, "msm_groupnorm_nchw_pool_f32: bad arguments (1..%d levels)", GP_MAXL);
+    if (opt(MSM_OPT_GN_POOL) == 0) {
+        if (int rc = msm_groupnorm_apply_nchw_f32(x, stats, gamma, beta, y, B, H * W, C, groups, eps, relu, stream)) return rc;
+        return msm_pool_mask_taps(y, B, H, W, n_levels, th, tw, out, zero_buf, zero_count, stream);
+    }
+    GnPoolLevels lv;
+    lv.n = n_levels;
+    for (int l = 0; l < GP_MAXL; ++l) {
+        if (l < n_levels) {
+            MSM_REQUIRE(out[l] && th[l] > 0 && tw[l] > 0 && H % th[l] == 0 && W % tw[l] == 0 && H / th[l] == W / tw[l],
+                        "msm_groupnorm_nchw_pool_f32: level %d (%dx%d) is not an integer reduction of %dx%d", l, th[l], tw[l], H, W);
+            const int p = H / th[l];
+            MSM_REQUIRE(p == 2 || p == 4 || p == 8, "msm_groupnorm_nchw_pool_f32: ratio %d not in {2, 4, 8}", p);
+            MSM_REQUIRE((((uintptr_t)out[l]) & 15) == 0, "msm_groupnorm_nchw_pool_f32: misaligned output");
+            lv.lg[l] = p == 2 ? 1 : (p == 4 ? 2 : 3); lv.th[l] = th[l]; lv.tw[l] = tw[l]; lv.out[l] = out[l];
+        } else {
+            lv.lg[l] = 1; lv.th[l] = lv.tw[l] = 0; lv.out[l] = nullptr;
+        }
+    }
+    dim3 grid(cdiv(W, GP_TW), cdiv(H, GP_TH), B), block(GP_T);
+    MSM_REQUIRE(grid.y <= 65535 && grid.z <= 65535, "msm_groupnorm_nchw_pool_f32: %dx%d x %d images exceeds the grid", H, W, B);
+    hipLaunchKernelGGL(gn_apply_nchw_pool_kernel, grid, block, 0, (hipStream_t)stream, x, stats, gamma, beta, y, lv, H, W, groups, eps, relu,
+                       zero_buf, zero_count);
+    MSM_CHECK_LAUNCH("msm_groupnorm_nchw_pool_f32");
+    return MSM_OK;
+}
+
 extern "C" int msm_pos_embed_sine(float* out, int H, int W, int npf, int64_t s_c, int64_t s_p, const float* add_c,
                                   float temperature, float scale, void* stream) {
     MSM_REQUIRE(out && H > 0 && W > 0 && npf > 0, "msm_pos_embed_sine: bad arguments");
diff --git a/unseenobjectswithmeanshift_amd/meta_arch.py b/unseenobjectswithmeanshift_amd/meta_arch.py
--- a/unseenobjectswithmeanshift_amd/meta_arch.py
+++ b/unseenobjectswithmeanshift_amd/meta_arch.py
@@ -138,6 +138,8 @@
         kw = {}
         if getattr(self.predictor, "folded_mask_features", False) and _accepts(self.pixel_decoder.forward_features, "folded"):
             kw["folded"] = True
+            if hasattr(self.predictor, "pool_request") and _accepts(self.pixel_decoder.forward_features, "pool_request"):
+                kw["pool_request"] = self.predictor.pool_request
         mask_features, _, multi_scale_features = self.pixel_decoder.forward_features(features, **kw)
         if final_topk and _accepts(self.predictor.forward, "final_topk"):
             predictions = self.predictor(multi_scale_features, mask_features, mask, final_topk=final_topk)
diff --git a/unseenobjectswithmeanshift_amd/modeling.py b/unseenobjectswithmeanshift_amd/modeling.py
--- a/unseenobjectswithmeanshift_amd/modeling.py
+++ b/unseenobjectswithmeanshift_amd/modeling.py
@@ -52,8 +52,9 @@
 
 class FoldedMaskFeatures:
 
-    def __init__(self, act, weight, bias, materialize):
+    def __init__(self, act, weight, bias, materialize, pooled=None):
         self.act, self.weight, self.bias = act, weight, bias
+        self.pooled = pooled
         self._materialize = materialize
         self._tensor = None
 
@@ -381,7 +382,8 @@
 
     @staticmethod
     def _poolable_sizes(act, sizes):
-        Hm, Wm = int(act.shape[2]), int(act.shape[3])
+        shape = getattr(act, "shape", act)
+        Hm, Wm = int(shape[2]), int(shape[3])
         out = []
         for (th, tw) in sizes:
             if (int(th), int(tw)) not in out and Hm % th == 0 and Wm % tw == 0 and Hm // th == Wm // tw and Hm // th in (2, 4, 8):
@@ -390,6 +392,23 @@
 
     def _keys_f16(self):
         return self.attention_dtype == "bf16" and self.attention_keys == "f16" and 2 * self.query_feat.weight.shape[1] == 512
+
+    def _pool_plan(self, act_shape, sizes, Qn):
+        full, L = self.aux_outputs, self.num_layers
+        if not (self.pooled_attention_masks and (not full or self.pooled_attention_masks == "always") and int(act_shape[1]) == 64 and L > 0):
+            return None
+        want_sizes = self._poolable_sizes(act_shape, sizes)
+        if not want_sizes:
+            return None
+        fuse_masks = bool(self.fused_head_masks) and self.tails_dtype in ("bf16", "f16") and not self._tails_hl_for("heads") and not full \
+            and self.lp_pooled_masks != "x3"
+        return want_sizes, Qn * (L + 1 if fuse_masks else 1), fuse_masks
+
+    def pool_request(self, act_shape, sizes):
+        if not (self.folded_mask_features and self.fused_tails and self.fold_kv and int(act_shape[1]) < self.query_feat.weight.shape[1]):
+            return None
+        plan = self._pool_plan(act_shape, [(int(h), int(w)) for h, w in sizes], int(self.query_feat.weight.shape[0]))
+        return None if plan is None else plan[:2]
 
     def _kv_one(self, x, w, cc):
         c, cw = cc
@@ -453,17 +472,19 @@
             fm_params = [t for t in (mask_features.weight, mask_features.bias) if t is not None]
             wf, bf, ncol = self._folded_head(mask_features)
             mlp[-1] = (wf, bf)
+            handed = mask_features.pooled
             mask_features = mask_features.act
-            if self.pooled_attention_masks and (not full or self.pooled_attention_masks == "always") and ncol == 64 and mask_features.shape[1] == 64:
-                want_sizes = self._poolable_sizes(mask_features, sizes)
-                if want_sizes and L > 0:
-                    fuse_masks = bool(self.fused_head_masks) and self.tails_dtype in ("bf16", "f16") and not self._tails_hl_for("heads") and not full \
-                        and self.lp_pooled_masks != "x3"
-                    Bq, Qn = int(out.shape[0]), int(out.shape[1])
-                    outs, flags = ops.pool_mask_taps(mask_features, want_sizes, zero_rows=Qn * (L + 1 if fuse_masks else 1))
-                    ra_all = flags.view(-1)[:Bq * Qn * (L + 1 if fuse_masks else 1)].view(-1, Bq, Qn)
-                    ra0 = ra_all[0]
-                    pooled = dict(zip(want_sizes, outs))
+            Bq, Qn = int(out.shape[0]), int(out.shape[1])
+            plan = self._pool_plan(mask_features.shape, sizes, Qn) if ncol == 64 else None
+            if plan is not None:
+                want_sizes, rows, fuse_masks = plan
+                if handed is not None and list(handed[0]) == want_sizes and handed[2] is not None and tuple(handed[2].shape) == (Bq, rows):
+                    outs, flags = handed[1], handed[2]
+                else:
+                    outs, flags = ops.pool_mask_taps(mask_features, want_sizes, zero_rows=rows)
+                ra_all = flags.view(-1)[:Bq * rows].view(-1, Bq, Qn)
+                ra0 = ra_all[0]
+                pooled = dict(zip(want_sizes, outs))
         dn = self.decoder_norm
         pred_cls, pred_mask = [], []
         topk_out = []
@@ -1133,7 +1154,7 @@
                 src = layer.forward_tokens(src, lvl_pos, ss, starts)
         return src, shapes, fpn_stats
 
-    def _fpn_mask_features(self, features, up_tok, up_hw, fpn_stats, folded=False):
+    def _fpn_mask_features(self, features, up_tok, up_hw, fpn_stats, folded=False, pool_request=None):
         C = self.conv_dim
         B = up_tok.shape[0]
         x = features[self.in_features[0]].float().contiguous()
@@ -1168,6 +1189,12 @@
                     ops.groupnorm_tokens(y, self.layer_1.norm.weight, self.layer_1.norm.bias, H, W, groups=32, relu=True,
                                          eps=self.layer_1.norm.eps), wm, self.mask_features.bias).view(B, self.mask_dim, H, W)
             if folded:
+                req = pool_request((B, C, H, W)) if (pool_request is not None and W % 4 == 0) else None
+                if req:
+                    want_sizes, rows = req
+                    act, outs, flags = ops.groupnorm_nchw_pool(y, y_stats, self.layer_1.norm.weight, self.layer_1.norm.bias, H, W, want_sizes,
+                                                               groups=32, eps=self.layer_1.norm.eps, relu=True, zero_rows=rows)
+                    return FoldedMaskFeatures(act, wm, self.mask_features.bias, literal, pooled=(list(want_sizes), outs, flags))
                 act = ops.groupnorm_nchw(y, y_stats, self.layer_1.norm.weight, self.layer_1.norm.bias, groups=32,
                                          eps=self.layer_1.norm.eps, relu=True).view(B, C, H, W)
                 return FoldedMaskFeatures(act, wm, self.mask_features.bias, literal)
@@ -1179,7 +1206,7 @@
         return mask_features
 
     @torch.no_grad()
-    def forward_features(self, features, folded=False):
+    def forward_features(self, features, folded=False, pool_request=None):
         C = self.conv_dim
         src, shapes, fpn_stats = self._encode(features)
         B = src.shape[0]
@@ -1188,5 +1215,8 @@
             out.append(src[:, o:o + h * w].view(B, h, w, C).permute(0, 3, 1, 2))
             o += h * w
         up_tok = src[:, o - shapes[-1][0] * shapes[-1][1]:]
-        mask_features = self._fpn_mask_features(features, up_tok, shapes[-1], fpn_stats, folded)
+        want = None
+        if folded and pool_request is not None:
+            want = lambda act_shape: pool_request(act_shape, shapes[:self.maskformer_num_feature_levels])
+        mask_features = self._fpn_mask_features(features, up_tok, shapes[-1], fpn_stats, folded, want)
         return mask_features, out[0], out[:self.maskformer_num_feature_levels]
diff --git a/unseenobjectswithmeanshift_amd/ops.py b/unseenobjectswithmeanshift_amd/ops.py
--- a/unseenobjectswithmeanshift_amd/ops.py
+++ b/unseenobjectswithmeanshift_amd/ops.py
@@ -278,6 +278,25 @@
                                             1 if relu else 0, _stream())
     check(rc, "msm_groupnorm_apply_nchw_f32")
     return y
+
+
+def groupnorm_nchw_pool(x, stats, gamma, beta, H, W, sizes, *, groups=32, eps=1e-5, relu=False, zero_rows=0):
+    _c(x, "x"), _c(stats, "stats", torch.float64), _c(gamma, "gamma"), _c(beta, "beta")
+    B, HW, C = x.shape
+    if C != 64 or HW != H * W or not 1 <= len(sizes) <= 4:
+        raise RuntimeError("groupnorm_nchw_pool needs a (B, H*W, 64) token map and 1..4 target sizes")
+    y = torch.empty((B, C, H, W), device=x.device, dtype=torch.float32)
+    outs = [torch.empty((B, int(th) * int(tw), 64), device=x.device, dtype=torch.float32) for th, tw in sizes]
+    n = len(sizes)
+    ths = (ctypes.c_int32 * n)(*[int(s[0]) for s in sizes])
+    tws = (ctypes.c_int32 * n)(*[int(s[1]) for s in sizes])
+    ptrs = (ctypes.c_void_p * n)(*[o.data_ptr() for o in outs])
+    flags = torch.empty((B, int(zero_rows)), device=x.device, dtype=torch.int32) if zero_rows else None
+    rc = lib().msm_groupnorm_nchw_pool_f32(_p(x), _p(stats), _p(gamma), _p(beta), _p(y), B, int(H), int(W), C, int(groups), float(eps),
+                                           1 if relu else 0, n, ctypes.cast(ths, ctypes.c_void_p), ctypes.cast(tws, ctypes.c_void_p),
+                                           ctypes.cast(ptrs, ctypes.c_void_p), _p(flags), B * int(zero_rows), _stream())
+    check(rc, "msm_groupnorm_nchw_pool_f32")
+    return y, outs, flags
 
 
 def groupnorm_stats(x, stats=None):
```

Result: faster. 3926 images/sec (median of 6 runs) (+1.9%).
